# carrenD/Medical-Cross-Modality-Domain-Adaptation

Hardware: AMD Instinct MI355X
Metric: training slices/sec (256x256x3, B=16/GPU) joint segmenter+GAN step (1 dis update on B MR + B CT, clip, 1 gen update on B CT) (higher is better)
Workload: dtype f32; 1 GPU; BASELINE configs[3]: train_gan.py --phase train-gan joint step, B=16/GPU per domain, f32, dropout .75, mask critic on; global_batch=16, per_gpu_batch=16, parallelism=dp1, step_capture=False

## Files before the change

### include/pnp_hip.h

```cpp
#ifndef PNP_HIP_H
#define PNP_HIP_H

#include <stddef.h>
#include <stdint.h>

#ifdef __cplusplus
extern "C" {
#endif

#define PNP_OK 0
#define PNP_EINVAL (-1)
#define PNP_ELAUNCH (-2)
#define PNP_EWORKSPACE (-3)
#define PNP_ECOMM (-4)

#define PNP_DTYPE_F32 0
#define PNP_DTYPE_BF16 1
#define PNP_DTYPE_F64 2

#define PNP_PAD_ZERO 0
#define PNP_PAD_SYMMETRIC 1

int pnp_abi_version(void);
const char* pnp_last_error(void);
int pnp_device_info(int device, int* cu_count, int* clock_khz, int* lds_bytes, char* arch, int arch_len);

#define PNP_PROF_CONV_FWD 1
#define PNP_PROF_CONV_DGRAD 2
#define PNP_PROF_CONV_WGRAD 4
#define PNP_PROF_CONV_DIRECT 8
typedef struct pnp_prof_row {
    char name[128];
    int64_t launches;
    double ms, flops, bytes;
} pnp_prof_row;
int pnp_prof_enable(int32_t mask);
int pnp_prof_summary(pnp_prof_row* rows, int32_t max_rows);

typedef struct pnp_conv_geom {
    int32_t N, H, W, C;
    int32_t K, R, S;
    int32_t OH, OW;
    int32_t stride, dil;
    int32_t pad_t, pad_l;
    int32_t pad_mode;
    int32_t dtype;
} pnp_conv_geom;

int pnp_conv2d_fwd(const float* x, const float* w, float* y, const pnp_conv_geom* g,
                   float keep_prob, uint64_t seed, uint32_t stream_id, void* stream);
size_t pnp_conv2d_fwd_workspace_bytes(const pnp_conv_geom* g);
int pnp_conv2d_fwd_ws(const float* x, const float* w, float* y, const pnp_conv_geom* g,
                      float keep_prob, uint64_t seed, uint32_t stream_id,
                      void* workspace, size_t workspace_bytes, void* stream);

int32_t pnp_conv2d_fwd_stats_parts(const pnp_conv_geom* g);
int pnp_conv2d_fwd_stats(const float* x, const float* w, float* y, const pnp_conv_geom* g,
                         float keep_prob, uint64_t seed, uint32_t stream_id,
                         const float* shift , float* parts, size_t parts_bytes, void* stream);
int32_t pnp_conv2d_fwd_stats_ws_parts(const pnp_conv_geom* g);
int pnp_conv2d_fwd_stats_ws(const float* x, const float* w, float* y, const pnp_conv_geom* g,
                            float keep_prob, uint64_t seed, uint32_t stream_id,
                            const float* shift , float* parts, size_t parts_bytes,
                            void* workspace, size_t workspace_bytes, void* stream);
int32_t pnp_conv2d_wino_chosen(const pnp_conv_geom* g, int32_t kind);
#define PNP_ROUTE_IGEMM 0
#define PNP_ROUTE_N16 1
#define PNP_ROUTE_NARROW 2
#define PNP_ROUTE_WINO 3
#define PNP_ROUTE_X3D 4
#define PNP_ROUTE_X3S 5
#define PNP_ROUTE_PHASES 6
#define PNP_ROUTE_WINO_WGRAD 7
#define PNP_ROUTE_X3W 8
#define PNP_ROUTE_N16_WGRAD 9
#define PNP_ROUTE_WGD 10
#define PNP_ROUTE_RING 11
#define PNP_ROUTE_X3N 12
int32_t pnp_conv2d_route(const pnp_conv_geom* g, int32_t kind);
int32_t pnp_conv2d_wino_mode(int32_t mode);
int32_t pnp_conv2d_wino_tile(int32_t tile);
int32_t pnp_conv2d_wino_x3(int32_t mode);
int32_t pnp_conv2d_x3_direct(int32_t mode);
int32_t pnp_conv2d_x3_strided(int32_t mode);
int32_t pnp_conv2d_x3_wgrad(int32_t mode);
int32_t pnp_conv2d_x3_narrow(int32_t mode);
size_t pnp_conv2d_wino_filter_bytes(int32_t C, int32_t K);
int pnp_conv2d_wino_filter_bind(const float* w, int32_t kind, float* U, size_t bytes);
void pnp_weights_changed(const void* lo, const void* hi);
void pnp_conv2d_wino_filter_stats(int64_t* hits, int64_t* fills, int32_t reset);
int32_t pnp_conv2d_wino_wgrad_mode(int32_t mode);

int pnp_bn_fold(const float* gamma, const float* beta, const float* mean, const float* var, float* scale, float* shift,
                int32_t C, float eps, void* stream);
int pnp_conv2d_fwd_bn(const float* x, const float* w, float* y, const pnp_conv_geom* g,
                      float keep_prob, uint64_t seed, uint32_t stream_id,
                      const float* scale, const float* shift, const float* shortcut , int32_t Cs, float alpha,
                      void* stream);
int pnp_conv2d_fwd_bn_ws(const float* x, const float* w, float* y, const pnp_conv_geom* g,
                         float keep_prob, uint64_t seed, uint32_t stream_id,
                         const float* scale, const float* shift, const float* shortcut , int32_t Cs, float alpha,
                         void* workspace, size_t workspace_bytes, void* stream);

size_t pnp_conv2d_dgrad_workspace_bytes(const pnp_conv_geom* g);
int pnp_conv2d_dgrad(const float* dy, const float* w, float* dx, const pnp_conv_geom* g,
                     void* workspace, size_t workspace_bytes, void* stream);
int pnp_conv2d_dgrad_add(const float* dy, const float* w, const float* residual, float* dx, const pnp_conv_geom* g,
                         void* workspace, size_t workspace_bytes, void* stream);

size_t pnp_conv2d_wgrad_workspace_bytes(const pnp_conv_geom* g);
int pnp_conv2d_wgrad(const float* x, const float* dy, float* dw, const pnp_conv_geom* g,
                     void* workspace, size_t workspace_bytes, void* stream);
int pnp_conv2d_wgrad_acc(const float* x, const float* dy, float* dw, const pnp_conv_geom* g,
                         void* workspace, size_t workspace_bytes, void* stream);

int pnp_conv2d_fwd_naive(const float* x, const float* w, float* y, const pnp_conv_geom* g, void* stream);

int pnp_dropout(const float* x, float* y, size_t n, float keep_prob, uint64_t seed, uint32_t stream_id, void* stream);

size_t pnp_bn_workspace_bytes(int64_t P, int32_t C);
int pnp_bn_stats(const float* x, float* mean, float* var, int64_t P, int32_t C,
                 void* workspace, size_t workspace_bytes, void* stream);
int pnp_bn_stats_update(const float* x, float* mean, float* var, float* moving_mean, float* moving_var, int64_t P, int32_t C,
                        float decay, void* workspace, size_t workspace_bytes, void* stream);
int pnp_bn_stats_finish(float* parts, int32_t nparts, const float* shift, float* mean, float* var,
                        float* moving_mean, float* moving_var, int64_t P, int32_t C, float decay, void* stream);
int pnp_bn_update_moving(float* moving_mean, float* moving_var, const float* mean, const float* var,
                         int64_t P, int32_t C, float decay, void* stream);
int pnp_bn_apply(const float* x, const float* mean, const float* var, const float* gamma, const float* beta,
                 const float* shortcut, int32_t Cs, float* y, int64_t P, int32_t C, float eps, float alpha,
                 void* stream);
int pnp_bn_bwd(const float* dout, const float* out , const float* x, const float* mean, const float* var,
               const float* gamma, const float* beta , float* dx, float* dgamma, float* dbeta, float* dshortcut, int32_t Cs,
               int64_t P, int32_t C, float eps, float alpha, int32_t training,
               float keep_prob, uint64_t seed, uint32_t stream_id,
               void* workspace, size_t workspace_bytes, void* stream);
int pnp_bn_bwd_acc(const float* dout, const float* out , const float* x, const float* mean, const float* var,
                   const float* gamma, const float* beta , float* dx, float* dgamma, float* dbeta, float* dgamma_acc, float* dbeta_acc,
                   float* dshortcut, int32_t Cs, int64_t P, int32_t C, float eps, float alpha, int32_t training,
                   float keep_prob, uint64_t seed, uint32_t stream_id,
                   void* workspace, size_t workspace_bytes, void* stream);
int pnp_bn_bwd_reduce(const float* dout, const float* out , const float* x, const float* mean, const float* var,
                      const float* gamma , const float* beta , float* dgamma, float* dbeta, int64_t P, int32_t C, float eps, float alpha,
                      void* workspace, size_t workspace_bytes, void* stream);
int pnp_bn_bwd_apply(const float* dout, const float* out , const float* x, const float* mean, const float* var,
                     const float* gamma, const float* beta , const float* dgamma, const float* dbeta, float* dx, float* dshortcut, int32_t Cs,
                     int64_t P, int64_t P_norm, int32_t C, float eps, float alpha, int32_t training,
                     float keep_prob, uint64_t seed, uint32_t stream_id, void* stream);


int pnp_maxpool2_fwd(const float* x, float* y, int32_t N, int32_t H, int32_t W, int32_t C, void* stream);
int pnp_maxpool2_bwd(const float* x, const float* dy, float* dx, int32_t N, int32_t H, int32_t W, int32_t C, void* stream);

int pnp_ps_fwd(const float* x, float* y, int32_t N, int32_t A, int32_t B, int32_t r, int32_t nc, void* stream);
int pnp_ps_bwd(const float* dy, float* dx, int32_t N, int32_t A, int32_t B, int32_t r, int32_t nc, void* stream);

int pnp_sympad_fwd(const float* x, float* xp, int32_t N, int32_t H, int32_t W, int32_t C, int32_t p, void* stream);
int pnp_sympad_bwd(const float* dxp, float* dx, int32_t N, int32_t H, int32_t W, int32_t C, int32_t p, void* stream);

int pnp_ps_pad_fwd(const float* x, float* xp, int32_t N, int32_t A, int32_t B, int32_t r, int32_t nc, int32_t p, void* stream);
int pnp_ps_pad_bwd(const float* dxp, float* dx, int32_t N, int32_t A, int32_t B, int32_t r, int32_t nc, int32_t p, void* stream);

size_t pnp_seg_loss_workspace_bytes(int64_t P, int32_t ncls);
int pnp_seg_loss_fwd(const float* logits, const float* y, float* out, int64_t P, int32_t ncls,
                     float miu_cross, float miu_dice, void* workspace, size_t workspace_bytes, void* stream);
int pnp_seg_loss_bwd(const float* logits, const float* y, float* dlogits, int64_t P, int32_t ncls,
                     float miu_cross, float miu_dice, float gscale,
                     const void* workspace, size_t workspace_bytes, void* stream);
int pnp_seg_loss_bwd_norm(const float* logits, const float* y, float* dlogits, int64_t P, int64_t P_norm, int32_t ncls,
                          float miu_cross, float miu_dice, float gscale,
                          const void* workspace, size_t workspace_bytes, void* stream);
int pnp_softmax_argmax(const float* logits, float* prob , int64_t* label, int64_t P, int32_t ncls, void* stream);
int pnp_dice_eval(const int64_t* label, const float* y, float* out, int64_t P, int32_t ncls,
                  void* workspace, size_t workspace_bytes, void* stream);

int pnp_label_decomp(const float* label, float* onehot, int64_t P, int32_t ncls, void* stream);
int pnp_confusion_matrix(const float* y, const int64_t* pred, int64_t* compact_y, int64_t* cm, int64_t P, int32_t ncls, void* stream);
int pnp_edt3d_sq(const uint8_t* mask, float* dist_sq, int64_t X, int64_t Y, int64_t Z, float sx, float sy, float sz, void* stream);
size_t pnp_surface_workspace_bytes(int64_t X, int64_t Y, int64_t Z, int32_t ncls);
int pnp_surface_distances(const int32_t* pred, const int32_t* gt, int64_t X, int64_t Y, int64_t Z, int32_t ncls, float sx, float sy,
                          float sz, double* out, void* workspace, size_t workspace_bytes, void* stream);
int pnp_gp_interpolate(const float* a, const float* b, float* out, float* eps, int64_t B, int64_t n, uint64_t seed, uint32_t stream_id,
                       void* stream);
size_t pnp_gp_workspace_bytes(int64_t B, int64_t n);
int pnp_gp_penalty(float* g, int64_t B, int64_t n, float coef, float gscale, float* norms, float* penalty, void* workspace,
// ... 187 lines not shown
```

### medical-cross-modality-domain-adaptation_amd/_lib.py

```python
import ctypes
import os

import torch

from ctypes import POINTER, c_char_p, c_double, c_float, c_int, c_int32, c_int64, c_size_t, c_uint32, c_uint64, c_void_p

_HERE = os.path.dirname(os.path.abspath(__file__))
LIB_PATH = os.environ.get("PNP_LIB") or os.path.join(_HERE, "libpnp_hip.so")

PAD_ZERO = 0
PAD_SYMMETRIC = 1
OPT_CHUNK = 1024
DTYPE_F32, DTYPE_BF16, DTYPE_F64 = 0, 1, 2
COMM_ID_BYTES = 128
(ROUTE_IGEMM, ROUTE_N16, ROUTE_NARROW, ROUTE_WINO, ROUTE_X3D, ROUTE_X3S, ROUTE_PHASES,
 ROUTE_WINO_WGRAD, ROUTE_X3W, ROUTE_N16_WGRAD, ROUTE_WGD, ROUTE_RING, ROUTE_X3N) = range(13)
ABI_VERSION = 4


class ConvGeom(ctypes.Structure):
    _fields_ = [(n, c_int32) for n in
                ("N", "H", "W", "C", "K", "R", "S", "OH", "OW", "stride", "dil", "pad_t", "pad_l", "pad_mode", "dtype")]

    def key(self):
        return tuple(getattr(self, f) for f, _ in self._fields_)


class ProfRow(ctypes.Structure):
    _fields_ = [("name", ctypes.c_char * 128), ("launches", c_int64), ("ms", ctypes.c_double), ("flops", ctypes.c_double),
                ("bytes", ctypes.c_double)]


class AugVolume(ctypes.Structure):
    _fields_ = [("image", c_void_p), ("label", c_void_p), ("X", c_int32), ("Y", c_int32), ("Z", c_int32), ("fill", c_float)]


class AugSample(ctypes.Structure):
    _fields_ = [("volume", c_int32), ("frame", c_int32), ("m", c_float * 6)]


class AugSampleZ(ctypes.Structure):
    _fields_ = [("volume", c_int32), ("frame", c_int32), ("dz", c_float), ("m", c_float * 6)]


class AugSampleW(ctypes.Structure):
    _fields_ = [("volume", c_int32), ("frame", c_int32), ("dz", c_float), ("m", c_float * 6), ("gain", c_float), ("bias", c_float),
                ("noise", c_float), ("seed", c_uint32), ("warp", c_int32)]


PROF_CONV_FWD, PROF_CONV_DGRAD, PROF_CONV_WGRAD, PROF_CONV_DIRECT = 1, 2, 4, 8


class PnpError(RuntimeError):
    pass


_F = c_void_p
_G = POINTER(ConvGeom)

PROTOTYPES = {
    "pnp_abi_version": (c_int, []),
    "pnp_last_error": (c_char_p, []),
    "pnp_device_info": (c_int, [c_int, POINTER(c_int), POINTER(c_int), POINTER(c_int), c_char_p, c_int]),
    "pnp_prof_enable": (c_int, [c_int32]),
    "pnp_prof_summary": (c_int, [POINTER(ProfRow), c_int32]),
    "pnp_conv2d_fwd": (c_int, [_F, _F, _F, _G, c_float, c_uint64, c_uint32, c_void_p]),
    "pnp_conv2d_dgrad_workspace_bytes": (c_size_t, [_G]),
    "pnp_conv2d_dgrad": (c_int, [_F, _F, _F, _G, c_void_p, c_size_t, c_void_p]),
    "pnp_conv2d_dgrad_add": (c_int, [_F, _F, _F, _F, _G, c_void_p, c_size_t, c_void_p]),
    "pnp_conv2d_wgrad_workspace_bytes": (c_size_t, [_G]),
    "pnp_conv2d_wgrad": (c_int, [_F, _F, _F, _G, c_void_p, c_size_t, c_void_p]),
    "pnp_conv2d_wgrad_acc": (c_int, [_F, _F, _F, _G, c_void_p, c_size_t, c_void_p]),
    "pnp_conv2d_fwd_workspace_bytes": (c_size_t, [_G]),
    "pnp_conv2d_fwd_ws": (c_int, [_F, _F, _F, _G, c_float, c_uint64, c_uint32, c_void_p, c_size_t, c_void_p]),
    "pnp_conv2d_fwd_stats_parts": (c_int32, [_G]),
    "pnp_conv2d_fwd_stats": (c_int, [_F, _F, _F, _G, c_float, c_uint64, c_uint32, _F, _F, c_size_t, c_void_p]),
    "pnp_bn_stats_finish": (c_int, [_F, c_int32, _F, _F, _F, _F, _F, c_int64, c_int32, c_float, c_void_p]),
    "pnp_bn_fold": (c_int, [_F, _F, _F, _F, _F, _F, c_int32, c_float, c_void_p]),
    "pnp_conv2d_fwd_bn": (c_int, [_F, _F, _F, _G, c_float, c_uint64, c_uint32, _F, _F, _F, c_int32, c_float, c_void_p]),
    "pnp_conv2d_fwd_bn_ws": (c_int, [_F, _F, _F, _G, c_float, c_uint64, c_uint32, _F, _F, _F, c_int32, c_float, c_void_p, c_size_t, c_void_p]),
    "pnp_conv2d_fwd_stats_ws_parts": (c_int32, [_G]),
    "pnp_conv2d_fwd_stats_ws": (c_int, [_F, _F, _F, _G, c_float, c_uint64, c_uint32, _F, _F, c_size_t, c_void_p, c_size_t, c_void_p]),
    "pnp_conv2d_wino_chosen": (c_int32, [_G, c_int32]),
    "pnp_conv2d_route": (c_int32, [_G, c_int32]),
    "pnp_conv2d_wino_mode": (c_int32, [c_int32]),
    "pnp_conv2d_wino_wgrad_mode": (c_int32, [c_int32]),
    "pnp_conv2d_wino_tile": (c_int32, [c_int32]),
    "pnp_conv2d_wino_x3": (c_int32, [c_int32]),
    "pnp_conv2d_x3_direct": (c_int32, [c_int32]),
    "pnp_conv2d_x3_strided": (c_int32, [c_int32]),
    "pnp_conv2d_x3_wgrad": (c_int32, [c_int32]),
    "pnp_conv2d_x3_narrow": (c_int32, [c_int32]),
    "pnp_conv2d_wino_filter_bytes": (c_size_t, [c_int32, c_int32]),
    "pnp_conv2d_wino_filter_bind": (c_int, [c_void_p, c_int32, c_void_p, c_size_t]),
    "pnp_weights_changed": (None, [c_void_p, c_void_p]),
    "pnp_conv2d_wino_filter_stats": (None, [POINTER(c_int64), POINTER(c_int64), c_int32]),
    "pnp_conv2d_fwd_naive": (c_int, [_F, _F, _F, _G, c_void_p]),
    "pnp_dropout": (c_int, [_F, _F, c_size_t, c_float, c_uint64, c_uint32, c_void_p]),
    "pnp_bn_workspace_bytes": (c_size_t, [c_int64, c_int32]),
    "pnp_bn_stats": (c_int, [_F, _F, _F, c_int64, c_int32, c_void_p, c_size_t, c_void_p]),
    "pnp_bn_stats_update": (c_int, [_F, _F, _F, _F, _F, c_int64, c_int32, c_float, c_void_p, c_size_t, c_void_p]),
    "pnp_bn_update_moving": (c_int, [_F, _F, _F, _F, c_int64, c_int32, c_float, c_void_p]),
    "pnp_bn_apply": (c_int, [_F, _F, _F, _F, _F, _F, c_int32, _F, c_int64, c_int32, c_float, c_float, c_void_p]),
    "pnp_bn_bwd": (c_int, [_F, _F, _F, _F, _F, _F, _F, _F, _F, _F, _F, c_int32, c_int64, c_int32, c_float, c_float, c_int32,
                           c_float, c_uint64, c_uint32, c_void_p, c_size_t, c_void_p]),
    "pnp_bn_bwd_acc": (c_int, [_F, _F, _F, _F, _F, _F, _F, _F, _F, _F, _F, _F, _F, c_int32, c_int64, c_int32, c_float, c_float, c_int32,
                               c_float, c_uint64, c_uint32, c_void_p, c_size_t, c_void_p]),
    "pnp_bn_bwd_reduce": (c_int, [_F, _F, _F, _F, _F, _F, _F, _F, _F, c_int64, c_int32, c_float, c_float, c_void_p, c_size_t, c_void_p]),
    "pnp_bn_bwd_apply": (c_int, [_F, _F, _F, _F, _F, _F, _F, _F, _F, _F, _F, c_int32, c_int64, c_int64, c_int32, c_float, c_float, c_int32,
                                 c_float, c_uint64, c_uint32, c_void_p]),
    "pnp_maxpool2_fwd": (c_int, [_F, _F, c_int32, c_int32, c_int32, c_int32, c_void_p]),
    "pnp_maxpool2_bwd": (c_int, [_F, _F, _F, c_int32, c_int32, c_int32, c_int32, c_void_p]),
    "pnp_ps_fwd": (c_int, [_F, _F, c_int32, c_int32, c_int32, c_int32, c_int32, c_void_p]),
    "pnp_ps_bwd": (c_int, [_F, _F, c_int32, c_int32, c_int32, c_int32, c_int32, c_void_p]),
    "pnp_sympad_fwd": (c_int, [_F, _F, c_int32, c_int32, c_int32, c_int32, c_int32, c_void_p]),
    "pnp_sympad_bwd": (c_int, [_F, _F, c_int32, c_int32, c_int32, c_int32, c_int32, c_void_p]),
    "pnp_ps_pad_fwd": (c_int, [_F, _F, c_int32, c_int32, c_int32, c_int32, c_int32, c_int32, c_void_p]),
    "pnp_ps_pad_bwd": (c_int, [_F, _F, c_int32, c_int32, c_int32, c_int32, c_int32, c_int32, c_void_p]),
    "pnp_seg_loss_workspace_bytes": (c_size_t, [c_int64, c_int32]),
    "pnp_seg_loss_fwd": (c_int, [_F, _F, _F, c_int64, c_int32, c_float, c_float, c_void_p, c_size_t, c_void_p]),
    "pnp_seg_loss_bwd": (c_int, [_F, _F, _F, c_int64, c_int32, c_float, c_float, c_float, c_void_p, c_size_t, c_void_p]),
    "pnp_seg_loss_bwd_norm": (c_int, [_F, _F, _F, c_int64, c_int64, c_int32, c_float, c_float, c_float, c_void_p, c_size_t, c_void_p]),
    "pnp_softmax_argmax": (c_int, [_F, _F, c_void_p, c_int64, c_int32, c_void_p]),
    "pnp_dice_eval": (c_int, [c_void_p, _F, _F, c_int64, c_int32, c_void_p, c_size_t, c_void_p]),
    "pnp_adam_step": (c_int, [_F, _F, _F, _F, c_size_t, _F, c_void_p, c_float, c_float, c_float, c_float, c_int32, c_void_p]),
    "pnp_rmsprop_step": (c_int, [_F, _F, _F, c_size_t, _F, c_void_p, c_float, c_float, c_float, c_void_p]),
    "pnp_momentum_step": (c_int, [_F, _F, _F, c_size_t, _F, c_void_p, c_float, c_float, c_void_p]),
    "pnp_clip": (c_int, [_F, c_size_t, c_void_p, c_float, c_float, c_void_p]),
    "pnp_l2_loss": (c_int, [_F, c_size_t, _F, _F, c_void_p, c_size_t, c_void_p]),
    "pnp_reduce_workspace_bytes": (c_size_t, [c_size_t]),
    "pnp_critic_input_fwd": (c_int, [_F, c_int32, c_int32, _F, c_int32, _F, c_int32, _F, c_int32, _F, c_int32, _F, c_int64, c_void_p]),
    "pnp_critic_input_bwd": (c_int, [_F, _F, c_int32, c_int32, _F, c_int32, _F, c_int32, _F, c_int32, _F, c_int32, c_int64, c_void_p]),
    "pnp_critic_input_ps_fwd": (c_int, [_F, c_int32, c_int32, _F, c_int32, _F, c_int32, _F, c_int32, _F, c_int32, _F, c_int32, c_int32, c_int32,
                                        c_int32, c_void_p]),
    "pnp_critic_input_ps_bwd": (c_int, [_F, _F, c_int32, c_int32, _F, c_int32, _F, c_int32, _F, c_int32, _F, c_int32, c_int32, c_int32, c_int32,
                                        c_int32, c_void_p]),
    "pnp_axpby": (c_int, [_F, _F, c_size_t, c_float, c_float, c_void_p]),
    "pnp_add": (c_int, [_F, _F, _F, c_size_t, c_void_p]),
    "pnp_softmax_entropy_workspace_bytes": (c_size_t, [c_int64, c_int32]),
    "pnp_softmax_entropy": (c_int, [_F, c_int64, c_int32, c_float, _F, _F, c_void_p, c_size_t, c_void_p]),
    "pnp_signed_distance_2d_workspace_bytes": (c_size_t, [c_int32, c_int32, c_int32, c_int32, c_uint32]),
    "pnp_signed_distance_2d": (c_int, [_F, c_int32, c_int32, c_int32, c_int32, c_uint32, _F, c_void_p, c_size_t, c_void_p]),
    "pnp_boundary_loss_workspace_bytes": (c_size_t, [c_int64, c_int32]),
    "pnp_boundary_loss": (c_int, [_F, _F, c_int64, c_int32, c_int32, c_float, _F, _F, c_void_p, c_size_t, c_void_p]),
    "pnp_pseudo_label_loss_workspace_bytes": (c_size_t, [c_int64, c_int32]),
    "pnp_pseudo_label_loss": (c_int, [_F, _F, c_int64, c_int32, c_uint32, c_float, _F, c_void_p, _F, _F, c_void_p, c_void_p, c_size_t, c_void_p]),
    "pnp_pseudo_label_update_workspace_bytes": (c_size_t, [c_int64, c_int32]),
    "pnp_pseudo_label_update": (c_int, [c_void_p, _F, c_int64, c_int32, c_double, c_float, _F, _F, c_void_p, c_size_t, c_void_p]),
    "pnp_fda_workspace_bytes": (c_size_t, [c_int32, c_int32, c_int32, c_int32, c_int32, c_int32]),
    "pnp_fda_amplitude_swap": (c_int, [_F, c_int32, _F, c_int32, c_int32, c_int32, c_int32, c_void_p, c_void_p, _F, c_void_p, c_size_t, c_void_p]),
    "pnp_wgan_loss": (c_int, [_F, _F, _F, _F, c_int32, c_float, c_float, c_float, c_float, _F, c_void_p]),
    "pnp_fill": (c_int, [_F, c_size_t, c_float, c_void_p]),
    "pnp_label_decomp": (c_int, [_F, _F, c_int64, c_int32, c_void_p]),
    "pnp_confusion_matrix": (c_int, [_F, c_void_p, c_void_p, c_void_p, c_int64, c_int32, c_void_p]),
    "pnp_edt3d_sq": (c_int, [c_void_p, _F, c_int64, c_int64, c_int64, c_float, c_float, c_float, c_void_p]),
    "pnp_surface_workspace_bytes": (c_size_t, [c_int64, c_int64, c_int64, c_int32]),
    "pnp_surface_distances": (c_int, [c_void_p, c_void_p, c_int64, c_int64, c_int64, c_int32, c_float, c_float, c_float, c_void_p, c_void_p,
                                      c_size_t, c_void_p]),
    "pnp_gp_interpolate": (c_int, [_F, _F, _F, _F, c_int64, c_int64, c_uint64, c_uint32, c_void_p]),
    "pnp_gp_workspace_bytes": (c_size_t, [c_int64, c_int64]),
    "pnp_gp_penalty": (c_int, [_F, c_int64, c_int64, c_float, c_float, _F, _F, c_void_p, c_size_t, c_void_p]),
    "pnp_bn_dbl_bwd_workspace_bytes": (c_size_t, [c_int64, c_int32]),
    "pnp_bn_dbl_bwd": (c_int, [_F, _F, _F, _F, _F, _F, _F, _F, c_int32, _F, _F, _F, c_int64, c_int32, c_float, c_float, c_float, c_uint64,
                               c_uint32, c_void_p, c_size_t, c_void_p]),
    "pnp_bn_moments": (c_int, [_F, _F, c_void_p, c_int32, c_void_p]),
    "pnp_bn_from_moments": (c_int, [c_void_p, c_int32, _F, _F, c_int32, c_void_p]),
    "pnp_cast_bf16": (c_int, [_F, c_void_p, c_size_t, c_void_p]),
    "pnp_filter_bf16": (c_int, [_F, c_void_p, c_void_p, c_int32, c_int32, c_int32, c_int32, c_void_p]),
    "pnp_conv2d_bf16r_served": (c_int32, [_G, c_int32]),
    "pnp_conv2d_fwd_bf16r_stats_parts": (c_int32, [_G]),
    "pnp_conv2d_fwd_bf16r": (c_int, [c_void_p, c_void_p, _F, c_void_p, _G, c_float, c_uint64, c_uint32, _F, _F, c_size_t, _F, _F, _F, c_int32,
                                     c_float, c_void_p]),
    "pnp_conv2d_dgrad_bf16r": (c_int, [c_void_p, c_void_p, _F, _F, c_void_p, _G, c_void_p]),
    "pnp_bn_apply_h": (c_int, [_F, _F, _F, _F, _F, _F, c_int32, _F, c_void_p, c_int64, c_int32, c_float, c_float, c_void_p]),
    "pnp_bn_bwd_acc_h": (c_int, [_F, _F, _F, _F, _F, _F, _F, _F, c_void_p, _F, _F, _F, _F, _F, c_int32, c_int64, c_int32, c_float, c_float,
                                 c_int32, c_float, c_uint64, c_uint32, c_void_p, c_size_t, c_void_p]),
    "pnp_bn_bwd_apply_h": (c_int, [_F, _F, _F, _F, _F, _F, _F, _F, _F, _F, c_void_p, _F, c_int32, c_int64, c_int64, c_int32, c_float, c_float,
                                   c_int32, c_float, c_uint64, c_uint32, c_void_p]),
    "pnp_dropout_h": (c_int, [_F, _F, c_void_p, c_size_t, c_float, c_uint64, c_uint32, c_void_p]),
# ... 87 lines not shown
```

### medical-cross-modality-domain-adaptation_amd/csrc/conv_common.h

```cpp
#pragma once
#include "pnp_common.h"

namespace pnpconv {

constexpr int BK = 32;
constexpr int NTHREADS = 256;

struct ConvArgs {
    const float* x;
    const float* w;
    float* y;
    int N, H, W, C, K, R, S, OH, OW, stride, dil, pad_t, pad_l, pad_mode;
    int ups;
    int M;
    int Kred;
    int OHW;
    int nblk_m, nblk_n;
    int gn;
    int nsplit, chunks_per_split;
    long long split_stride;
    uint32_t drop_thresh, drop_key;
    float drop_keep;
    int do_drop;
    const pnp_step_params* sp;
    uint32_t drop_sid;
    int xcd_swizzle;
    unsigned x_bytes, w_bytes;
    int stagger;
    int o_s, o_H, o_W, o_h0, o_w0;
    const float* ep_scale;
    const float* ep_shift;
    const float* ep_res;
    int ep_cs;
    float ep_alpha;
    int dtype;
    float* stat_ws;
    const float* stat_shift;
    const float* res_add;
    int accumulate;
    int ow_sh, ohw_sh;
    int ph_st, ph_pa, ph_pb, ph_S;
    unsigned short* y_h;
};

__device__ __forceinline__ void split_row(const ConvArgs& a, int m, int& n, int& oh, int& ow) {
    if (a.ohw_sh >= 0) {
        n = m >> a.ohw_sh;
        const int rem = m & (a.OHW - 1);
        oh = rem >> a.ow_sh;
        ow = rem & (a.OW - 1);
    } else {
        n = m / a.OHW;
        const int rem = m - n * a.OHW;
        oh = rem / a.OW;
        ow = rem - oh * a.OW;
    }
}

__device__ __forceinline__ float bn_epilogue(const ConvArgs& a, float v, int m, int n) {
    v = fmaf(v, a.ep_scale[n], a.ep_shift[n]);
    if (a.ep_res) {
        const int cs = n - ((a.K - a.ep_cs) >> 1);
        if ((unsigned)cs < (unsigned)a.ep_cs) v += a.ep_res[(size_t)m * a.ep_cs + cs];
    }
    return (a.ep_alpha >= 0.f && v < 0.f) ? v * a.ep_alpha : v;
}

__device__ __forceinline__ size_t out_row(const ConvArgs& a, int m, bool scatter) {
    if (!scatter) return (size_t)m * a.K;
    int n, oh, ow;
    split_row(a, m, n, oh, ow);
    return ((size_t)(n * a.o_H + a.o_h0 + oh * a.o_s) * a.o_W + a.o_w0 + ow * a.o_s) * a.K;
}

template <bool UPS>
__device__ __forceinline__ bool map_coord(int v, int H, int ups, int sym, int& i) {
    const int vs = v < 0 ? -1 - v : (v >= H ? 2 * H - 1 - v : v);
    const int vv = sym ? vs : v;
    if constexpr (UPS) {
        const int q = vv / ups;
        i = q;
        return (vv >= 0) & (q * ups == vv) & (q < H);
    } else {
        i = vv;
        return (unsigned)vv < (unsigned)H;
    }
}

__device__ __forceinline__ int xcd_remap(int bid, int nblk) {
    const int NX = 8;
    int q = nblk / NX, r = nblk % NX;
    int xcd = bid % NX, idx = bid / NX;
    int base = (xcd < r) ? xcd * (q + 1) : r * (q + 1) + (xcd - r) * q;
    return base + idx;
}

__device__ __forceinline__ void tile_coords(int bid, int nblk_m, int nblk_n, int gn, int& mt, int& nt) {
    if (gn <= 0 || gn >= nblk_n) { mt = bid / nblk_n; nt = bid - mt * nblk_n; return; }
    const int span = nblk_m * gn;
    const int sc = bid / span, rem = bid - sc * span;
    const int left = nblk_n - sc * gn;
    const int width = left < gn ? left : gn;
    mt = rem / width;
    nt = sc * gn + rem - mt * width;
}

template <int TM, int TN>
struct Acc {
    f32x16 v[TM][TN];
    __device__ __forceinline__ void zero() {
#pragma unroll
        for (int i = 0; i < TM; ++i)
#pragma unroll
            for (int j = 0; j < TN; ++j)
#pragma unroll
                for (int e = 0; e < 16; ++e) v[i][j][e] = 0.f;
    }
};

typedef unsigned int u32x4 __attribute__((ext_vector_type(4)));
typedef const float __attribute__((address_space(4))) pnp_cfloat;
constexpr unsigned OOB = 0xFFFFFF00u;

__device__ __forceinline__ __amdgpu_buffer_rsrc_t make_rsrc(const float* p, unsigned bytes) {
    return __builtin_amdgcn_make_buffer_rsrc(const_cast<float*>(p), 0, bytes, 0x00020000);
}
__device__ __forceinline__ f32x4 bload4(__amdgpu_buffer_rsrc_t r, unsigned off) {
    return __builtin_bit_cast(f32x4, __builtin_amdgcn_raw_buffer_load_b128(r, off, 0, 0));
}
__device__ __forceinline__ float bload1(__amdgpu_buffer_rsrc_t r, unsigned off) {
    return __builtin_bit_cast(float, __builtin_amdgcn_raw_buffer_load_b32(r, off, 0, 0));
}
__device__ __forceinline__ void bstore1(__amdgpu_buffer_rsrc_t r, unsigned off, float v) {
    __builtin_amdgcn_raw_buffer_store_b32(__builtin_bit_cast(unsigned, v), r, off, 0, 0);
}


template <int TM, int TN>
__device__ __forceinline__ void conv_epilogue(const ConvArgs& a, const Acc<TM, TN>& acc, float* __restrict__ yout, int m0, int n0, int wm0,
                                              int wn0, int lane, int part, bool first_split = true) {
    const float* __restrict__ res = first_split ? a.res_add : nullptr;
    const int l31 = lane & 31, h = lane >> 5;
    const bool scatter = a.o_s != 0 && a.nsplit == 1;
// ... 117 lines not shown
        for (int tm = 0; tm < TM; ++tm)
#pragma unroll
            for (int tn = 0; tn < TN; ++tn) {
                const int n = n0 + wn0 + tn * 32 + l31;
#pragma unroll
                for (int r = 0; r < 16; ++r) {
                    const int m = mbase + tm * 32 + (r & 3) + 8 * (r >> 2);
                    const bool ok = (m < a.Kred) & (n < a.K);
                    old.v[tm][tn][r] = out[ok ? (size_t)m * a.K + n : 0];
                }
            }
#pragma unroll
        for (int tm = 0; tm < TM; ++tm)
#pragma unroll
            for (int tn = 0; tn < TN; ++tn)
#pragma unroll
                for (int r = 0; r < 16; ++r) o.v[tm][tn][r] += old.v[tm][tn][r];
    }
#pragma unroll
    for (int tm = 0; tm < TM; ++tm)
#pragma unroll
        for (int tn = 0; tn < TN; ++tn) {
            const int n = n0 + wn0 + tn * 32 + l31;
#pragma unroll
            for (int r = 0; r < 16; ++r) {
                const int m = mbase + tm * 32 + (r & 3) + 8 * (r >> 2);
                if ((m < a.Kred) & (n < a.K)) out[(size_t)m * a.K + n] = o.v[tm][tn][r];
            }
        }
}

constexpr unsigned OOB2 = 0x80000000u;

__device__ __forceinline__ f32x4 bload4s(__amdgpu_buffer_rsrc_t r, unsigned voff, int soff) {
    return __builtin_bit_cast(f32x4, __builtin_amdgcn_raw_buffer_load_b128(r, voff, soff, 0));
}

__device__ __forceinline__ float bload1s(__amdgpu_buffer_rsrc_t r, unsigned voff, int soff) {
    return __builtin_bit_cast(float, __builtin_amdgcn_raw_buffer_load_b32(r, voff, soff, 0));
}

bool launch_taps_bf16(const ConvArgs& a, int tile, int kind, dim3 grid, hipStream_t st);
bool launch_wgrad_bf16(const ConvArgs& a, int tile, dim3 grid, hipStream_t st);
constexpr int kWgradBf16rChunk = 64;
bool launch_wgrad_bf16r(const ConvArgs& a, int tile, dim3 grid, hipStream_t st);
int wgrad_bf16r_tile(const pnp_conv_geom* g);
struct DgradPhase {
    int pa, pb, T, U, h0, w0, I, J, pad_t, pad_l;
    size_t wt_off;
};
int plan_phases(const pnp_conv_geom* g, DgradPhase* ph);
pnp_conv_geom phase_geom(const pnp_conv_geom* g, const DgradPhase& p);
bool n16_geom_ok(const pnp_conv_geom* g);
bool n16_wgrad_ok(const pnp_conv_geom* g);
int launch_n16_fwd(const ConvArgs& a, int kind, hipStream_t st);
int n16_wgrad_blocks(const pnp_conv_geom* g);
int launch_n16_wgrad(const ConvArgs& a, float* part, hipStream_t st);
bool narrow_fwd_ok(const pnp_conv_geom* g);
int launch_narrow(const float* x, const float* w, float* y, const pnp_conv_geom* g, const ConvArgs& a, hipStream_t st);
bool wgd_ok(const pnp_conv_geom* g);
size_t wgd_workspace_bytes(const pnp_conv_geom* g);
int wgd_blocks(const pnp_conv_geom* g);
int launch_wgd(const float* x, const float* dy, float* part, const pnp_conv_geom* g, const ConvArgs& a, hipStream_t st);
bool x3d_chosen(const pnp_conv_geom* g);
int x3d_stats_parts(const pnp_conv_geom* g);
size_t x3d_filter_bytes(int C, int K);
int launch_x3_direct(const ConvArgs& a, int kind, bool flip_transpose, void* ws, size_t ws_bytes, hipStream_t st);
bool x3s_chosen(const pnp_conv_geom* g, int kind);
size_t x3s_filter_bytes(const pnp_conv_geom* g);
int launch_x3_strided(const ConvArgs& a, const pnp_conv_geom* g, int kind, void* ws, size_t ws_bytes, hipStream_t st);
int x3d_route_mode();
bool x3w_chosen(const pnp_conv_geom* g);
size_t x3w_workspace_bytes(const pnp_conv_geom* g);
int launch_x3_wgrad(const float* x, const float* dy, float* dw, const pnp_conv_geom* g, int accumulate, void* ws, size_t ws_bytes, hipStream_t st);
bool x3n_chosen(const pnp_conv_geom* g, int kind);
size_t x3n_filter_bytes(int kind);
int launch_x3_narrow(const ConvArgs& a, int kind, void* ws, size_t ws_bytes, hipStream_t st);
struct WinoQuery {
    int tile;
    size_t ws_bytes;
    int stats_parts;
};
WinoQuery wino_query(const pnp_conv_geom* g);
int launch_wino(const ConvArgs& a, int kind, bool flip_transpose, void* ws, size_t ws_bytes, hipStream_t st);
WinoQuery wino_wgrad_query(const pnp_conv_geom* g);
int launch_wino_wgrad(const ConvArgs& a, float* dw, int accumulate, void* ws, size_t ws_bytes, hipStream_t st);
#ifndef PNP_X3_SW
#define PNP_X3_SW 32
#endif
constexpr int X3_SW = PNP_X3_SW;
static_assert(X3_SW == 16 || X3_SW == 32, "stage width");
bool wino_x3_dims_ok(int T, int C, int K);
int launch_wino_gemm_x3(const unsigned short* V3, const unsigned short* U3, float* Mm, int T, int C, int K, int npos, int sym, int gn, int xcd,
                        int nsplit, int stages_per_split, hipStream_t st);
inline double conv_flops(const ConvArgs& a) { return 2.0 * (double)a.M * a.K * a.Kred; }
inline double conv_bytes(const ConvArgs& a) {
    return 4.0 * ((double)a.N * a.H * a.W * a.C + (double)a.M * a.K + (double)a.Kred * a.K);
}
inline int prof_class(int kind) { return kind == 0 ? PNP_PROF_CONV_FWD : PNP_PROF_CONV_DGRAD; }

}
```

### medical-cross-modality-domain-adaptation_amd/csrc/conv_igemm.hip

```cpp
#include "conv_common.h"
#include "conv_mma.h"
#include "split_sum.h"

using namespace pnpconv;

#ifdef PNP_TRACE
constexpr int TRACE_WG = 512, TRACE_N = 192;
__device__ unsigned long long g_trace[TRACE_WG][TRACE_N];
#define PNP_TRACE_MARK(slot)                                                                             \
    do {                                                                                                 \
        const unsigned tr_ = blockIdx.x - (gridDim.x > 4352u ? 4096u : 0u);        \
        if (threadIdx.x == 0 && tr_ < (unsigned)TRACE_WG && (slot) < TRACE_N) g_trace[tr_][(slot)] = __builtin_readcyclecounter(); \
    } while (0)
extern "C" int pnp_debug_trace_read(void* host, size_t bytes) {
    if (bytes > sizeof(unsigned long long) * TRACE_WG * TRACE_N) bytes = sizeof(unsigned long long) * TRACE_WG * TRACE_N;
    return hipMemcpyFromSymbol(host, HIP_SYMBOL(g_trace), bytes, 0, hipMemcpyDeviceToHost) == hipSuccess ? 0 : -1;
}
#else
#define PNP_TRACE_MARK(slot) do { } while (0)
#endif

namespace {

template <int BN, bool VEC>
// ... 766 lines not shown
    Stage ring[DEPTH];
    int l_chunk = c_begin;
    auto gload = [&](Stage& st) {
#pragma unroll
        for (int i = 0; i < ANP; ++i) {
            if constexpr (UNI) {
                unsigned so[2];
#pragma unroll
                for (int h = 0; h < 2; ++h) {
                    const bool ok = ((unsigned)u_ih[i][h] < (unsigned)a.H) & ((unsigned)u_iw[i][h] < (unsigned)a.W);
                    so[h] = ok ? (unsigned)u_off[i][h] : OOB2;
                    u_iw[i][h] += step_w;
                    u_ih[i][h] += step_h;
                    u_off[i][h] += step_off;
                    const bool ww = u_iw[i][h] >= u_iw_lim;
                    u_iw[i][h] -= ww ? wrap_w : 0;
                    u_ih[i][h] += ww ? a.stride : 0;
                    u_off[i][h] += ww ? wrap_w_off : 0;
                    const bool hw = u_ih[i][h] >= u_ih_lim;
                    u_ih[i][h] -= hw ? wrap_h : 0;
                    u_off[i][h] += hw ? wrap_h_off : 0;
                }
                st.a[i] = bload4(rx, ((lane & 32) ? so[1] : so[0]) + lane_c);
                continue;
            }
            const bool ok = mok & ((unsigned)l_ih[i] < (unsigned)a.H) & ((unsigned)l_iw[i] < (unsigned)a.W);
            st.a[i] = bload4(rx, ok ? (unsigned)l_off[i] : OOB);
            l_iw[i] += step_w;
            l_ih[i] += step_h;
            l_off[i] += step_off;
            const bool ww = l_iw[i] >= iw_lim;
            l_iw[i] -= ww ? wrap_w : 0;
            l_ih[i] += ww ? a.stride : 0;
            l_off[i] += ww ? wrap_w_off : 0;
            const bool hw = l_ih[i] >= ih_lim;
            l_ih[i] -= hw ? wrap_h : 0;
            l_off[i] += hw ? wrap_h_off : 0;
        }
        const int soff = __builtin_amdgcn_readfirstlane(l_chunk * BK * a.K * 4);
#pragma unroll
        for (int i = 0; i < BNP; ++i) st.b[i] = bload4s(rw, boff[i], soff);
        l_chunk = (l_chunk + 1 < nchunks_total) ? l_chunk + 1 : nchunks_total;
    };
    auto lstore = [&](const Stage& st, float* An, float* Bn) {
#pragma unroll
        for (int i = 0; i < ANP; ++i) *reinterpret_cast<f32x4*>(An + (arow + ARP * i) * LDA + 4 * acol) = st.a[i];
#pragma unroll
        for (int i = 0; i < BNP; ++i) *reinterpret_cast<f32x4*>(Bn + (brow + BRP * i) * LDB + 4 * bcol) = st.b[i];
    };

    Acc<TM, TN> acc;
    acc.zero();
    if (nchunks > 0) {
#pragma unroll
        for (int d = 0; d < DEPTH; ++d) gload(ring[d]);
        lstore(ring[0], lds, lds + 2 * ASZ);
        __syncthreads();
        Frag<TM, TN, false, LDA, LDB> f0, f1;
        f0.load(lds, lds + 2 * ASZ, 0, wm0, wn0, lane);
        auto stage = [&](int j, Stage& fetch_into, const Stage& store_from, bool fetch) {
            const int cur = j & 1;
            const float* As = lds + cur * ASZ;
            const float* Bs = lds + 2 * ASZ + cur * BSZ;
            float* An = lds + (cur ^ 1) * ASZ;
            float* Bn = lds + 2 * ASZ + (cur ^ 1) * BSZ;
            PNP_MMA_STAGE(12, 4 * TM + 4 * TN, 4 * TM * TN, if (fetch) gload(fetch_into), lstore(store_from, An, Bn))
            f0.load(An, Bn, 0, wm0, wn0, lane);
        };
        const int nmain = (nchunks / DEPTH) * DEPTH;
        for (int j0 = 0; j0 < nmain; j0 += DEPTH) {
#pragma unroll
            for (int d = 0; d < DEPTH; ++d) stage(j0 + d, ring[d], ring[(d + 1) % DEPTH], true);
        }
        if (nchunks - nmain >= 1) stage(nmain, ring[0], ring[1], false);
    }

    wgrad_epilogue<TM, TN>(a, acc, a.y + (size_t)z * a.split_stride, mm0, n0, wm0, wn0, lane);
}

__global__ void bn_fold_kernel(const float* __restrict__ gamma, const float* __restrict__ beta, const float* __restrict__ mean,
                               const float* __restrict__ var, float* __restrict__ scale, float* __restrict__ shift, int C, float eps) {
    const int c = blockIdx.x * blockDim.x + threadIdx.x;
    if (c >= C) return;
    const float sc = gamma[c] * (1.0f / sqrtf(var[c] + eps));
    scale[c] = sc;
    shift[c] = beta[c] - mean[c] * sc;
}

__global__ void flip_transpose_phase_kernel(const float* __restrict__ w, float* __restrict__ wt, int R, int S, int C, int K, int st) {
    __shared__ float tile[32][33];
    const int r = blockIdx.z / S, sx = blockIdx.z - r * S;
    const int pa = r % st, pb = sx % st;
    const int T = (R - pa + st - 1) / st, U = (S - pb + st - 1) / st;
    int taps_before = 0;
    for (int a = 0; a < st; ++a)
        for (int b = 0; b < st; ++b)
            if (a * st + b < pa * st + pb) taps_before += ((R - a + st - 1) / st) * ((S - b + st - 1) / st);
    const int tf = T - 1 - r / st, uf = U - 1 - sx / st;
    const float* src = w + (size_t)blockIdx.z * C * K;
    float* dst = wt + ((size_t)taps_before + tf * U + uf) * K * C;
    const int c0 = blockIdx.y * 32, k0 = blockIdx.x * 32;
    const int tx = threadIdx.x & 31, ty = threadIdx.x >> 5;
    for (int i = ty; i < 32; i += 8) {
        int c = c0 + i, k = k0 + tx;
        tile[i][tx] = (c < C && k < K) ? src[(size_t)c * K + k] : 0.f;
    }
    __syncthreads();
    for (int i = ty; i < 32; i += 8) {
        int k = k0 + i, c = c0 + tx;
        if (k < K && c < C) dst[(size_t)k * C + c] = tile[tx][i];
    }
}

__global__ void flip_transpose_kernel(const float* __restrict__ w, float* __restrict__ wt, int R, int S, int C, int K) {
    __shared__ float tile[32][33];
    const int rs = blockIdx.z;
    const int r = rs / S, s = rs - r * S;
    const int rs_f = (R - 1 - r) * S + (S - 1 - s);
    const float* src = w + (size_t)rs * C * K;
    float* dst = wt + (size_t)rs_f * K * C;
    const int c0 = blockIdx.y * 32, k0 = blockIdx.x * 32;
    const int tx = threadIdx.x & 31, ty = threadIdx.x >> 5;
    for (int i = ty; i < 32; i += 8) {
        int c = c0 + i, k = k0 + tx;
        tile[i][tx] = (c < C && k < K) ? src[(size_t)c * K + k] : 0.f;
    }
    __syncthreads();
    for (int i = ty; i < 32; i += 8) {
        int k = k0 + i, c = c0 + tx;
        if (k < K && c < C) dst[(size_t)k * C + c] = tile[tx][i];
    }
}

__global__ void naive_conv_kernel(ConvArgs a) {
    size_t idx = (size_t)blockIdx.x * blockDim.x + threadIdx.x;
    const size_t total = (size_t)a.M * a.K;
    if (idx >= total) return;
    const int k = (int)(idx % a.K);
    const int m = (int)(idx / a.K);
    const int n = m / a.OHW;
    const int rem = m - n * a.OHW;
    const int oh = rem / a.OW, ow = rem - oh * a.OW;
    float acc = 0.f;
    for (int r = 0; r < a.R; ++r)
        for (int s = 0; s < a.S; ++s) {
            int ih = 0, iw = 0;
            if (!map_coord<true>(oh * a.stride - a.pad_t + r * a.dil, a.H, a.ups, a.pad_mode, ih)) continue;
            if (!map_coord<true>(ow * a.stride - a.pad_l + s * a.dil, a.W, a.ups, a.pad_mode, iw)) continue;
            const float* xp = a.x + ((size_t)(n * a.H + ih) * a.W + iw) * a.C;
            const float* wp = a.w + (size_t)((r * a.S + s) * a.C) * a.K + k;
            for (int c = 0; c < a.C; ++c) acc = fmaf(xp[c], wp[(size_t)c * a.K], acc);
        }
    a.y[idx] = acc;
}

__global__ void sympad_fwd_kernel(const float* __restrict__ x, float* __restrict__ xp, int N, int H, int W, int C, int p, int vec) {
    const int CV = vec ? (C >> 2) : C;
    const int Hp = H + 2 * p, Wp = W + 2 * p;
    const size_t total = (size_t)N * Hp * Wp * CV;
    const size_t gs = (size_t)gridDim.x * blockDim.x;
    for (size_t i = (size_t)blockIdx.x * blockDim.x + threadIdx.x; i < total; i += gs) {
        const int cv = (int)(i % CV);
        size_t q = i / CV;
        const int wp = (int)(q % Wp);
        q /= Wp;
        const int hp = (int)(q % Hp);
        const int n = (int)(q / Hp);
        int h = hp - p, w = wp - p;
        h = h < 0 ? -1 - h : (h >= H ? 2 * H - 1 - h : h);
// ... 522 lines not shown
    int route;
    size_t x3 = 0;
    DgradPhase ph[16];
    const int nph = plan_phases(g, ph);
    p.dws = dgrad_ws(g, d, ph, nph);
    const size_t b = p.dws.total;
    if (nph > 0) {
        route = x3s_chosen(g, 1) ? PNP_ROUTE_X3S : PNP_ROUTE_PHASES;
        if (route == PNP_ROUTE_X3S) x3 = x3s_filter_bytes(g);
    } else {
        if (!sym && n16_geom_ok(&d)) route = PNP_ROUTE_N16;
        else if (g->stride == 1 && narrow_fwd_ok(&d)) route = PNP_ROUTE_NARROW;
        else if (plain && x3d_chosen(&d)) route = PNP_ROUTE_X3D;
        else if (plain && x3n_chosen(g, 1)) route = PNP_ROUTE_X3N;
        else route = PNP_ROUTE_IGEMM;
        if (route == PNP_ROUTE_X3D) x3 = x3d_filter_bytes(d.C, d.K);
        if (route == PNP_ROUTE_X3N) x3 = x3n_filter_bytes(1);
    }
    p.ws_bytes = b > x3 ? b : x3;
    p.add(route, p.ws_bytes);
    return p;
}

static ConvPlan plan_wgrad(const pnp_conv_geom* g) {
    ConvPlan p{};
    const WinoQuery wq = wino_wgrad_query(g);
    p.tile = wq.tile;
    if (p.tile) p.add(PNP_ROUTE_WINO_WGRAD, wq.ws_bytes);
    if (x3w_chosen(g)) p.add(PNP_ROUTE_X3W, x3w_workspace_bytes(g));
    const size_t nout = (size_t)g->R * g->S * g->C * g->K;
    const bool wgd = wgd_ok(g);
    const int nsplit = ring_split(g);
    if (p.ncand) p.ws_bytes = p.cand[0].need;
    else if (n16_wgrad_ok(g)) p.ws_bytes = (size_t)n16_wgrad_blocks(g) * nout * sizeof(float);
    else {
        const size_t mfma_ws = nsplit <= 1 ? 0 : (size_t)nsplit * nout * sizeof(float);
        p.ws_bytes = (wgd && wgd_workspace_bytes(g) > mfma_ws) ? wgd_workspace_bytes(g) : mfma_ws;
    }
    if (n16_wgrad_ok(g)) p.add(PNP_ROUTE_N16_WGRAD, p.ws_bytes);
    if (wgd) p.add(PNP_ROUTE_WGD, wgd_workspace_bytes(g));
    p.add(PNP_ROUTE_RING, 0, nsplit);
    return p;
}

static void set_dropout(ConvArgs& a, float keep_prob, uint64_t seed, uint32_t stream_id) {
    if (keep_prob >= 1.f) return;
    a.do_drop = 1;
    a.drop_keep = keep_prob;
    a.drop_key = pnp_drop_key(seed, stream_id);
    a.drop_thresh = pnp_drop_thresh(keep_prob);
    a.sp = pnp_step_params_ptr(); a.drop_sid = stream_id;
}

static int launch_fwd_cand(const ConvPlan::Cand& c, ConvArgs& a, const pnp_conv_geom* g, void* ws, size_t ws_bytes, hipStream_t st) {
    switch (c.route) {
    case PNP_ROUTE_N16: return launch_n16_fwd(a, 0, st);
    case PNP_ROUTE_NARROW: return launch_narrow(a.x, a.w, a.y, g, a, st);
    case PNP_ROUTE_WINO: return launch_wino(a, 0, false, ws, ws_bytes, st);
    case PNP_ROUTE_X3D: return launch_x3_direct(a, 0, false, ws, ws_bytes, st);
    case PNP_ROUTE_X3S: return launch_x3_strided(a, g, 0, ws, ws_bytes, st);
    case PNP_ROUTE_X3N: return launch_x3_narrow(a, 0, ws, ws_bytes, st);
    default: return launch_fwd<0>(a, st, c.need ? (float*)ws : nullptr, ws_bytes, c.nsplit);
    }
}

static ConvPlan plan_of(const pnp_conv_geom* g, int kind) { return kind == 0 ? plan_fwd(g, EP_WS) : (kind == 2 ? plan_wgrad(g) : plan_dgrad(g)); }

extern "C" {

int32_t pnp_conv2d_route(const pnp_conv_geom* g, int32_t kind) {
    if (!g || check_geom(g, "pnp_conv2d_route") != PNP_OK) return -1;
    return plan_of(g, kind).cand[0].route;
}

int32_t pnp_conv2d_wino_chosen(const pnp_conv_geom* g, int32_t kind) {
    if (!g || check_geom(g, "pnp_conv2d_wino_chosen") != PNP_OK) return 0;
    return plan_of(g, kind).tile;
}

size_t pnp_conv2d_fwd_workspace_bytes(const pnp_conv_geom* g) { return g ? plan_fwd(g, EP_WS).ws_bytes : 0; }
size_t pnp_conv2d_dgrad_workspace_bytes(const pnp_conv_geom* g) { return g ? plan_dgrad(g).ws_bytes : 0; }
size_t pnp_conv2d_wgrad_workspace_bytes(const pnp_conv_geom* g) { return g ? plan_wgrad(g).ws_bytes : 0; }

int pnp_conv2d_fwd(const float* x, const float* w, float* y, const pnp_conv_geom* g, float keep_prob, uint64_t seed,
                   uint32_t stream_id, void* stream) {
    return pnp_conv2d_fwd_ws(x, w, y, g, keep_prob, seed, stream_id, nullptr, 0, stream);
}

int pnp_conv2d_fwd_ws(const float* x, const float* w, float* y, const pnp_conv_geom* g, float keep_prob, uint64_t seed,
                      uint32_t stream_id, void* workspace, size_t workspace_bytes, void* stream) {
    if (int e = check_geom(g, "pnp_conv2d_fwd")) return e;
    PNP_REQUIRE(x && w && y, "pnp_conv2d_fwd: null pointer");
    PNP_REQUIRE(keep_prob > 0.f, "pnp_conv2d_fwd: keep_prob must be > 0");
    ConvArgs a = make_args(x, w, y, g);
    set_dropout(a, keep_prob, seed, stream_id);
    return launch_fwd_cand(plan_fwd(g, EP_WS).pick(workspace, workspace_bytes), a, g, workspace, workspace_bytes, (hipStream_t)stream);
}

static int fwd_stats_impl(const float* x, const float* w, float* y, const pnp_conv_geom* g, float keep_prob, uint64_t seed,
                          uint32_t stream_id, const float* shift, float* parts, size_t parts_bytes, void* workspace, size_t workspace_bytes,
                          void* stream, unsigned ep) {
    if (int e = check_geom(g, "pnp_conv2d_fwd_stats")) return e;
    PNP_REQUIRE(x && w && y && parts, "pnp_conv2d_fwd_stats: null pointer");
    PNP_REQUIRE(keep_prob > 0.f, "pnp_conv2d_fwd_stats: keep_prob must be > 0");
    const ConvPlan p = plan_fwd(g, ep);
    const ConvPlan::Cand& c = p.cand[0];
    PNP_REQUIRE(c.need == 0 || (workspace && workspace_bytes >= c.need), "pnp_conv2d_fwd_stats_ws: workspace too small (pnp_conv2d_fwd_workspace_bytes)");
    PNP_REQUIRE(p.stats_parts > 0, "pnp_conv2d_fwd_stats: no epilogue statistics for this geometry (pnp_conv2d_fwd_stats_parts == 0)");
    if (parts_bytes < (size_t)p.stats_parts * 2 * g->K * sizeof(float)) {
        pnp_set_error("pnp_conv2d_fwd_stats: parts buffer too small (%zu < %zu)", parts_bytes, (size_t)p.stats_parts * 2 * g->K * sizeof(float));
        return PNP_EWORKSPACE;
    }
    ConvArgs a = make_args(x, w, y, g);
    set_dropout(a, keep_prob, seed, stream_id);
    a.stat_ws = parts;
    a.stat_shift = shift;
    return launch_fwd_cand(c, a, g, workspace, workspace_bytes, (hipStream_t)stream);
}

int32_t pnp_conv2d_fwd_stats_parts(const pnp_conv_geom* g) {
    return (g && check_geom(g, "pnp_conv2d_fwd_stats_parts") == PNP_OK) ? plan_fwd(g, EP_STATS).stats_parts : 0;
}

int pnp_conv2d_fwd_stats(const float* x, const float* w, float* y, const pnp_conv_geom* g, float keep_prob, uint64_t seed,
                         uint32_t stream_id, const float* shift, float* parts, size_t parts_bytes, void* stream) {
    return fwd_stats_impl(x, w, y, g, keep_prob, seed, stream_id, shift, parts, parts_bytes, nullptr, 0, stream, EP_STATS);
}

int32_t pnp_conv2d_fwd_stats_ws_parts(const pnp_conv_geom* g) {
    return (g && check_geom(g, "pnp_conv2d_fwd_stats_ws_parts") == PNP_OK) ? plan_fwd(g, EP_STATS | EP_WS).stats_parts : 0;
}

int pnp_conv2d_fwd_stats_ws(const float* x, const float* w, float* y, const pnp_conv_geom* g, float keep_prob, uint64_t seed,
                            uint32_t stream_id, const float* shift, float* parts, size_t parts_bytes, void* workspace,
                            size_t workspace_bytes, void* stream) {
    return fwd_stats_impl(x, w, y, g, keep_prob, seed, stream_id, shift, parts, parts_bytes, workspace, workspace_bytes, stream, EP_STATS | EP_WS);
}

int pnp_bn_fold(const float* gamma, const float* beta, const float* mean, const float* var, float* scale, float* shift, int32_t C,
                float eps, void* stream) {
    PNP_REQUIRE(gamma && beta && mean && var && scale && shift && C > 0, "pnp_bn_fold: bad argument");
    hipLaunchKernelGGL(bn_fold_kernel, dim3((unsigned)pnp_cdiv(C, 256)), dim3(256), 0, (hipStream_t)stream, gamma, beta, mean, var, scale,
                       shift, C, eps);
    PNP_CHECK_LAUNCH("bn_fold_kernel");
    return PNP_OK;
}

int pnp_conv2d_fwd_bn(const float* x, const float* w, float* y, const pnp_conv_geom* g, float keep_prob, uint64_t seed,
                      uint32_t stream_id, const float* scale, const float* shift, const float* shortcut, int32_t Cs, float alpha,
                      void* stream) {
    return pnp_conv2d_fwd_bn_ws(x, w, y, g, keep_prob, seed, stream_id, scale, shift, shortcut, Cs, alpha, nullptr, 0, stream);
}

int pnp_conv2d_fwd_bn_ws(const float* x, const float* w, float* y, const pnp_conv_geom* g, float keep_prob, uint64_t seed,
                         uint32_t stream_id, const float* scale, const float* shift, const float* shortcut, int32_t Cs, float alpha,
                         void* workspace, size_t workspace_bytes, void* stream) {
    if (int e = check_geom(g, "pnp_conv2d_fwd_bn")) return e;
    PNP_REQUIRE(x && w && y && scale && shift, "pnp_conv2d_fwd_bn: null pointer");
    PNP_REQUIRE(keep_prob > 0.f, "pnp_conv2d_fwd_bn: keep_prob must be > 0");
    if (shortcut) PNP_REQUIRE(Cs > 0 && Cs <= g->K && ((g->K - Cs) % 2) == 0, "pnp_conv2d_fwd_bn: bad shortcut channels");
    ConvArgs a = make_args(x, w, y, g);
    set_dropout(a, keep_prob, seed, stream_id);
    a.ep_scale = scale; a.ep_shift = shift; a.ep_res = shortcut; a.ep_cs = shortcut ? Cs : g->K; a.ep_alpha = alpha;
    return launch_fwd_cand(plan_fwd(g, EP_WS | EP_BN).pick(workspace, workspace_bytes), a, g, workspace, workspace_bytes, (hipStream_t)stream);
}

int pnp_conv2d_fwd_naive(const float* x, const float* w, float* y, const pnp_conv_geom* g, void* stream) {
    if (int e = check_geom(g, "pnp_conv2d_fwd_naive")) return e;
    ConvArgs a = make_args(x, w, y, g);
    const size_t total = (size_t)a.M * a.K;
    hipLaunchKernelGGL(naive_conv_kernel, dim3((unsigned)pnp_cdiv((long long)total, 256)), dim3(256), 0,
                       (hipStream_t)stream, a);
    PNP_CHECK_LAUNCH("naive_conv_kernel");
    return PNP_OK;
}

static int dgrad_impl(const float* dy, const float* w, float* dx, const pnp_conv_geom* g, void* workspace, size_t workspace_bytes, void* stream,
                      const float* residual) {
    if (int e = check_geom(g, "pnp_conv2d_dgrad")) return e;
    PNP_REQUIRE(dy && w && dx && workspace, "pnp_conv2d_dgrad: null pointer");
    const ConvPlan p = plan_dgrad(g);
    PNP_REQUIRE(workspace_bytes >= p.ws_bytes, "pnp_conv2d_dgrad: workspace too small");
    const bool sym = g->pad_mode == PNP_PAD_SYMMETRIC;
    if (sym) PNP_REQUIRE(g->pad_t == g->pad_l, "pnp_conv2d_dgrad: SYMMETRIC needs pad_t == pad_l");
    hipStream_t st = (hipStream_t)stream;
    const int route = p.cand[0].route;
    const pnp_conv_geom d = dgrad_as_conv(g);
    if (route == PNP_ROUTE_X3S) {
        ConvArgs a = make_args(dy, w, dx, g);
        if (int e = launch_x3_strided(a, g, 1, workspace, workspace_bytes, st)) return e;
        return residual ? pnp_axpby(residual, dx, (size_t)g->N * g->H * g->W * g->C, 1.f, 1.f, stream) : PNP_OK;
    }
    if (route == PNP_ROUTE_WINO || route == PNP_ROUTE_X3D || route == PNP_ROUTE_X3N) {
        ConvArgs a = make_args(dy, w, dx, &d);
        a.res_add = residual;
        if (route == PNP_ROUTE_X3N) return launch_x3_narrow(a, 1, workspace, workspace_bytes, st);
        return route == PNP_ROUTE_WINO ? launch_wino(a, 1, true, workspace, workspace_bytes, st)
                                       : launch_x3_direct(a, 1, true, workspace, workspace_bytes, st);
    }
    const DgradWs& dws = p.dws;
    float* wt = (float*)workspace;
    float* out = sym ? (float*)((char*)workspace + dws.filt) : dx;
    float* parts = (float*)((char*)workspace + dws.filt + dws.padded);
    auto split_ws = [&](int ns) { return ns > 1 ? parts : nullptr; };
    const dim3 tg((unsigned)pnp_cdiv(g->K, 32), (unsigned)pnp_cdiv(g->C, 32), (unsigned)(g->R * g->S));
    if (route == PNP_ROUTE_PHASES) {
        DgradPhase ph[16];
        const int nph = plan_phases(g, ph);
        hipLaunchKernelGGL(flip_transpose_phase_kernel, tg, dim3(256), 0, st, w, wt, g->R, g->S, g->C, g->K, g->stride);
        PNP_CHECK_LAUNCH("flip_transpose_phase_kernel");
        if (phases_in_one_launch(g, ph, nph)) {
            if (int e = launch_phase_group(dy, wt, out, g, ph, nph, d.OH, d.OW, st)) return e;
        } else {
            for (int i = 0; i < nph; ++i) {
                const DgradPhase& q = ph[i];
                if (q.I == 0 || q.J == 0) continue;
                const pnp_conv_geom dp = phase_geom(g, q);
                ConvArgs a = make_args(dy, wt + q.wt_off, out, &dp);
                a.o_s = g->stride; a.o_H = d.OH; a.o_W = d.OW; a.o_h0 = q.h0; a.o_w0 = q.w0;
                if (int e = launch_fwd<1>(a, st, split_ws(dws.nsplit[i]), dws.parts, dws.nsplit[i])) return e;
            }
        }
    } else {
        hipLaunchKernelGGL(flip_transpose_kernel, tg, dim3(256), 0, st, w, wt, g->R, g->S, g->C, g->K);
        PNP_CHECK_LAUNCH("flip_transpose_kernel");
        PNP_REQUIRE(d.pad_t >= 0 && d.pad_l >= 0, "pnp_conv2d_dgrad: forward padding exceeds the filter extent");
        ConvArgs a = make_args(dy, wt, out, &d);
        a.ups = g->stride;
        if (route == PNP_ROUTE_N16) {
            a.res_add = residual;
            return launch_n16_fwd(a, 1, st);
        }
        if (route == PNP_ROUTE_NARROW) {
            if (int e = launch_narrow(dy, wt, out, &d, a, st)) return e;
        } else {
            if (residual && !sym && g->stride == 1) {
                a.res_add = residual;
                residual = nullptr;
            }
            const int ns = dws.nsplit[0];
            if (int e = (g->stride > 1 ? launch_fwd<2>(a, st, split_ws(ns), dws.parts, ns) : launch_fwd<1>(a, st, split_ws(ns), dws.parts, ns))) return e;
        }
    }
    if (sym) {
        if (int e = pnp_sympad_bwd(out, dx, g->N, g->H, g->W, g->C, g->pad_t, stream)) return e;
    }
    return residual ? pnp_axpby(residual, dx, (size_t)g->N * g->H * g->W * g->C, 1.f, 1.f, stream) : PNP_OK;
}

int pnp_conv2d_dgrad(const float* dy, const float* w, float* dx, const pnp_conv_geom* g, void* workspace,
                     size_t workspace_bytes, void* stream) {
    return dgrad_impl(dy, w, dx, g, workspace, workspace_bytes, stream, nullptr);
}

int pnp_conv2d_dgrad_add(const float* dy, const float* w, const float* residual, float* dx, const pnp_conv_geom* g, void* workspace,
                         size_t workspace_bytes, void* stream) {
    PNP_REQUIRE(residual && residual != dx, "pnp_conv2d_dgrad_add: residual must be a tensor of its own");
    return dgrad_impl(dy, w, dx, g, workspace, workspace_bytes, stream, residual);
}

static int wgrad_impl(const float* x, const float* dy, float* dw, const pnp_conv_geom* g, void* workspace, size_t workspace_bytes, void* stream,
                      int accumulate) {
    if (int e = check_geom(g, "pnp_conv2d_wgrad")) return e;
    PNP_REQUIRE(x && dy && dw, "pnp_conv2d_wgrad: null pointer");
    ConvArgs a = make_args(x, dy, dw, g);
    a.accumulate = accumulate;
    a.w_bytes = (unsigned)((size_t)g->N * g->OH * g->OW * g->K * sizeof(float));
    hipStream_t st = (hipStream_t)stream;
    float* ws = (float*)workspace;
    if (!ws) workspace_bytes = 0;
    const size_t nout = (size_t)a.Kred * a.K;
    int nparts = 0;
    const ConvPlan::Cand c = plan_wgrad(g).pick(workspace, workspace_bytes);
    switch (c.route) {
    case PNP_ROUTE_WINO_WGRAD: return launch_wino_wgrad(a, dw, accumulate, workspace, workspace_bytes, st);
    case PNP_ROUTE_X3W: return launch_x3_wgrad(x, dy, dw, g, accumulate, workspace, workspace_bytes, st);
    case PNP_ROUTE_N16_WGRAD:
        if (int e = launch_n16_wgrad(a, ws, st)) return e;
        nparts = n16_wgrad_blocks(g);
        break;
    case PNP_ROUTE_WGD:
        if (int e = launch_wgd(x, dy, ws, g, a, st)) return e;
        nparts = wgd_blocks(g);
        break;
    default: {
        const RingTile t = ring_tile(a.K);
        if (!t.vecb) return launch_wgrad_tile<128, 32, 4, 1, false>(a, dw, ws, workspace_bytes, c.nsplit, st);
        if (t.bn == 128) return launch_wgrad_tile<128, 128, 2, 2, true>(a, dw, ws, workspace_bytes, c.nsplit, st);
        if (t.bn == 64) return launch_wgrad_tile<128, 64, 2, 2, true>(a, dw, ws, workspace_bytes, c.nsplit, st);
        return launch_wgrad_tile<128, 32, 4, 1, true>(a, dw, ws, workspace_bytes, c.nsplit, st);
    }
    }
    return split_sum::launch_sliced<1>(ws, dw, (int)nout, nparts, accumulate, st);
}

int pnp_conv2d_wgrad(const float* x, const float* dy, float* dw, const pnp_conv_geom* g, void* workspace,
                     size_t workspace_bytes, void* stream) {
    return wgrad_impl(x, dy, dw, g, workspace, workspace_bytes, stream, 0);
}

int pnp_conv2d_wgrad_acc(const float* x, const float* dy, float* dw, const pnp_conv_geom* g, void* workspace,
                         size_t workspace_bytes, void* stream) {
    return wgrad_impl(x, dy, dw, g, workspace, workspace_bytes, stream, 1);
}

static int wgrad_bf16r_plan(const pnp_conv_geom* g, int* bm, int* bn) {
    const int tile = wgrad_bf16r_tile(g);
    if (tile < 0) return 0;
// ... 79 lines not shown
```

### medical-cross-modality-domain-adaptation_amd/csrc/conv_small.hip

```cpp
#include "conv_common.h"

using namespace pnpconv;

namespace {

constexpr int TH = 8, TW = 32;
constexpr int PH = TH + 2, PW = TW + 2;

__device__ __forceinline__ f32x4 mfma16(float a, float b, f32x4 c) { return __builtin_amdgcn_mfma_f32_16x16x4f32(a, b, c, 0, 0, 0); }

template <int C, int LD>
__device__ __forceinline__ void load_patch(const ConvArgs& a, __amdgpu_buffer_rsrc_t rx, float* __restrict__ lds, int n, int oh0, int ow0, int t) {
    constexpr int CQ = C / 4;
    for (int i = t; i < PH * PW * CQ; i += 256) {
        const int pix = i / CQ, cq = i - pix * CQ;
        const int py = pix / PW, px = pix - py * PW;
        const int ih = oh0 - a.pad_t + py, iw = ow0 - a.pad_l + px;
        const bool ok = ((unsigned)ih < (unsigned)a.H) & ((unsigned)iw < (unsigned)a.W);
        const f32x4 v = bload4(rx, ok ? (unsigned)((((n * a.H + ih) * a.W + iw) * C + 4 * cq) * 4) : OOB);
        *reinterpret_cast<f32x4*>(lds + pix * LD + 4 * cq) = v;
    }
}

template <int C, int KIND>
__global__ void __launch_bounds__(256) conv_n16_kernel(ConvArgs a, int tiles_w, int tiles_per_wg) {
    constexpr int LD = C + 4, NH = C / 16;
    __shared__ __attribute__((aligned(16))) float lds[PH * PW * LD];
    const int t = threadIdx.x, lane = t & 63;
    const int wave = __builtin_amdgcn_readfirstlane(t >> 6);
    const int p = lane & 15, g = lane >> 4;
    const int n = blockIdx.z, oh0 = blockIdx.y * TH;
    const __amdgpu_buffer_rsrc_t rx = make_rsrc(a.x, a.x_bytes);

    float wreg[9][NH][4];
#pragma unroll
    for (int tap = 0; tap < 9; ++tap)
#pragma unroll
        for (int h = 0; h < NH; ++h)
#pragma unroll
            for (int j = 0; j < 4; ++j) wreg[tap][h][j] = a.w[(tap * C + 16 * h + 4 * g + j) * 16 + p];

    const int jt0 = blockIdx.x * tiles_per_wg;
    for (int jt = jt0; jt < jt0 + tiles_per_wg && jt < tiles_w; ++jt) {
        const int ow0 = jt * TW;
        __syncthreads();
        load_patch<C, LD>(a, rx, lds, n, oh0, ow0, t);
        __syncthreads();
        f32x4 acc[4];
#pragma unroll
        for (int q = 0; q < 4; ++q) acc[q] = f32x4{0.f, 0.f, 0.f, 0.f};
#pragma unroll
        for (int tap = 0; tap < 9; ++tap) {
            const int r = tap / 3, s = tap % 3;
#pragma unroll
            for (int q = 0; q < 4; ++q) {
                const int pix = (2 * wave + (q >> 1) + r) * PW + 16 * (q & 1) + p + s;
#pragma unroll
                for (int h = 0; h < NH; ++h) {
                    const f32x4 av = *reinterpret_cast<const f32x4*>(lds + pix * LD + 16 * h + 4 * g);
#pragma unroll
                    for (int j = 0; j < 4; ++j) acc[q] = mfma16(av[j], wreg[tap][h][j], acc[q]);
                }
            }
        }
        float ov[4][4];
        size_t oidx[4][4];
        bool ook[4][4];
#pragma unroll
        for (int q = 0; q < 4; ++q) {
            const int oh = oh0 + 2 * wave + (q >> 1);
#pragma unroll
            for (int i = 0; i < 4; ++i) {
                const int ow = ow0 + 16 * (q & 1) + 4 * g + i;
                ook[q][i] = oh < a.OH && ow < a.OW;
                const int m = ook[q][i] ? (n * a.OH + oh) * a.OW + ow : 0;
                oidx[q][i] = (size_t)m * 16 + p;
                float v = acc[q][i];
                if (a.do_drop) v = pnp_drop_keep((uint32_t)oidx[q][i], pnp_eff_drop_key(a.drop_key, a.sp, a.drop_sid), a.drop_thresh) ? v / a.drop_keep : 0.f;
                if (a.res_add) v += a.res_add[oidx[q][i]];
                if (a.ep_scale) v = bn_epilogue(a, v, m, p);
                ov[q][i] = v;
            }
        }
#pragma unroll
        for (int q = 0; q < 4; ++q)
#pragma unroll
            for (int i = 0; i < 4; ++i)
                if (ook[q][i]) a.y[oidx[q][i]] = ov[q][i];
    }
}

template <int C>
__global__ void __launch_bounds__(256) wgrad_n16_kernel(ConvArgs a, int tiles_w, int tiles_h, int ntiles) {
    constexpr int LD = (C == 16) ? 16 : 48, NC = C / 16, NT = 9 * NC;
    constexpr int LDSF = PH * PW * LD > NT * 256 ? PH * PW * LD : NT * 256;
    __shared__ __attribute__((aligned(16))) float lds[LDSF];
    const int t = threadIdx.x, lane = t & 63;
    const int wave = __builtin_amdgcn_readfirstlane(t >> 6);
    const int p = lane & 15, g = lane >> 4;
    const __amdgpu_buffer_rsrc_t rx = make_rsrc(a.x, a.x_bytes);
    const __amdgpu_buffer_rsrc_t rdy = make_rsrc(a.w, a.w_bytes);
    const int kg0 = blockIdx.y * 16;
    f32x4 acc[NT];
#pragma unroll
    for (int i = 0; i < NT; ++i) acc[i] = f32x4{0.f, 0.f, 0.f, 0.f};

    for (int tile = blockIdx.x; tile < ntiles; tile += gridDim.x) {
        const int jt = tile % tiles_w, rest = tile / tiles_w;
        const int it = rest % tiles_h, n = rest / tiles_h;
        const int oh0 = it * TH, ow0 = jt * TW;
        __syncthreads();
        load_patch<C, LD>(a, rx, lds, n, oh0, ow0, t);
        __syncthreads();
#pragma unroll 4
        for (int q = 0; q < 16; ++q) {
            const int row = 2 * wave + (q >> 3), col = 4 * (q & 7) + g;
            const int oh = oh0 + row, ow = ow0 + col;
            const bool ok = (oh < a.OH) & (ow < a.OW);
            const float dyv = bload1(rdy, ok ? (unsigned)((((n * a.OH + oh) * a.OW + ow) * a.K + kg0 + p) * 4) : OOB);
#pragma unroll
            for (int tap = 0; tap < 9; ++tap) {
                const int pix = (row + tap / 3) * PW + col + tap % 3;
#pragma unroll
                for (int c = 0; c < NC; ++c) {
                    const float xv = lds[pix * LD + 16 * c + p];
                    acc[tap * NC + c] = mfma16(xv, dyv, acc[tap * NC + c]);
                }
            }
        }
    }
    for (int w = 0; w < 4; ++w) {
        __syncthreads();
        if (wave == w) {
#pragma unroll
            for (int i = 0; i < NT; ++i) {
                f32x4* slot = reinterpret_cast<f32x4*>(lds + (i * 64 + lane) * 4);
                if (w == 0) *slot = acc[i];
                else {
                    f32x4 v = *slot;
#pragma unroll
                    for (int k = 0; k < 4; ++k) v[k] += acc[i][k];
                    *slot = v;
                }
            }
        }
    }
    __syncthreads();
    float* out = a.y + (size_t)blockIdx.x * (9 * C * a.K) + kg0;
    for (int e = t; e < NT * 64; e += 256) {
        const int i = e >> 6, l = e & 63;
        const f32x4 s = *reinterpret_cast<const f32x4*>(lds + (i * 64 + l) * 4);
        const int tap = i / NC, c = i - tap * NC, lp = l & 15, lg = l >> 4;
#pragma unroll
        for (int k = 0; k < 4; ++k) out[(size_t)(tap * C + 16 * c + 4 * lg + k) * a.K + lp] = s[k];
    }
}

__device__ __forceinline__ void load_patch3(const ConvArgs& a, __amdgpu_buffer_rsrc_t rx, float* __restrict__ lds, int n, int oh0, int ow0, int t) {
    for (int i = t; i < PH * PW; i += 256) {
        const int py = i / PW, px = i - py * PW;
        const int ih = oh0 - a.pad_t + py, iw = ow0 - a.pad_l + px;
        const bool ok = ((unsigned)ih < (unsigned)a.H) & ((unsigned)iw < (unsigned)a.W);
        const unsigned off = ok ? (unsigned)((((n * a.H + ih) * a.W + iw) * 3) * 4) : OOB;
        f32x4 v;
        v[0] = bload1(rx, off);
        v[1] = bload1(rx, ok ? off + 4u : OOB);
        v[2] = bload1(rx, ok ? off + 8u : OOB);
        v[3] = 0.f;
        *reinterpret_cast<f32x4*>(lds + i * 4) = v;
    }
}

template <int KIND>
__global__ void __launch_bounds__(256) conv_c3n16_kernel(ConvArgs a, int tiles_w, int tiles_per_wg) {
    __shared__ __attribute__((aligned(16))) float lds[PH * PW * 4];
    const int t = threadIdx.x, lane = t & 63;
    const int wave = __builtin_amdgcn_readfirstlane(t >> 6);
    const int p = lane & 15, g = lane >> 4;
    const int n = blockIdx.z, oh0 = blockIdx.y * TH;
    const __amdgpu_buffer_rsrc_t rx = make_rsrc(a.x, a.x_bytes);
    float wreg[7];
    int aoff[7];
#pragma unroll
    for (int i = 0; i < 7; ++i) {
        const int kk = 4 * i + g;
        const int tap = kk < 27 ? kk / 3 : 0, c = kk < 27 ? kk - 3 * (kk / 3) : 3;
        wreg[i] = kk < 27 ? a.w[kk * 16 + p] : 0.f;
        aoff[i] = ((tap / 3) * PW + tap % 3) * 4 + c;
    }
    const int jt0 = blockIdx.x * tiles_per_wg;
    for (int jt = jt0; jt < jt0 + tiles_per_wg && jt < tiles_w; ++jt) {
        const int ow0 = jt * TW;
        __syncthreads();
        load_patch3(a, rx, lds, n, oh0, ow0, t);
        __syncthreads();
#pragma unroll
        for (int q = 0; q < 4; ++q) {
            const int base = ((2 * wave + (q >> 1)) * PW + 16 * (q & 1) + p) * 4;
            f32x4 acc = {0.f, 0.f, 0.f, 0.f};
#pragma unroll
            for (int i = 0; i < 7; ++i) acc = mfma16(lds[base + aoff[i]], wreg[i], acc);
            const int oh = oh0 + 2 * wave + (q >> 1);
            float ov[4];
            size_t oidx[4];
            bool ook[4];
#pragma unroll
            for (int i = 0; i < 4; ++i) {
                const int ow = ow0 + 16 * (q & 1) + 4 * g + i;
                ook[i] = oh < a.OH && ow < a.OW;
                const int m = ook[i] ? (n * a.OH + oh) * a.OW + ow : 0;
                oidx[i] = (size_t)m * 16 + p;
                float v = acc[i];
                if (a.do_drop) v = pnp_drop_keep((uint32_t)oidx[i], pnp_eff_drop_key(a.drop_key, a.sp, a.drop_sid), a.drop_thresh) ? v / a.drop_keep : 0.f;
                if (a.res_add) v += a.res_add[oidx[i]];
                if (a.ep_scale) v = bn_epilogue(a, v, m, p);
                ov[i] = v;
            }
#pragma unroll
            for (int i = 0; i < 4; ++i)
                if (ook[i]) a.y[oidx[i]] = ov[i];
        }
    }
}

__global__ void __launch_bounds__(256) wgrad_c3n16_kernel(ConvArgs a, int tiles_w, int tiles_h, int ntiles) {
    __shared__ __attribute__((aligned(16))) float lds[PH * PW * 4 > 2 * 256 ? PH * PW * 4 : 2 * 256];
    const int t = threadIdx.x, lane = t & 63;
    const int wave = __builtin_amdgcn_readfirstlane(t >> 6);
    const int p = lane & 15, g = lane >> 4;
    const __amdgpu_buffer_rsrc_t rx = make_rsrc(a.x, a.x_bytes);
    const __amdgpu_buffer_rsrc_t rdy = make_rsrc(a.w, a.w_bytes);
    int aoff[2];
#pragma unroll
    for (int T = 0; T < 2; ++T) {
        const int mm = 16 * T + p;
        const int tap = mm < 27 ? mm / 3 : 0, c = mm < 27 ? mm - 3 * (mm / 3) : 3;
        aoff[T] = ((tap / 3) * PW + tap % 3) * 4 + c;
    }
    f32x4 acc[2] = {{0.f, 0.f, 0.f, 0.f}, {0.f, 0.f, 0.f, 0.f}};
    for (int tile = blockIdx.x; tile < ntiles; tile += gridDim.x) {
        const int jt = tile % tiles_w, rest = tile / tiles_w;
        const int it = rest % tiles_h, n = rest / tiles_h;
        const int oh0 = it * TH, ow0 = jt * TW;
        __syncthreads();
        load_patch3(a, rx, lds, n, oh0, ow0, t);
        __syncthreads();
#pragma unroll 4
        for (int q = 0; q < 16; ++q) {
            const int row = 2 * wave + (q >> 3), col = 4 * (q & 7) + g;
            const int oh = oh0 + row, ow = ow0 + col;
            const bool ok = (oh < a.OH) & (ow < a.OW);
            const float dyv = bload1(rdy, ok ? (unsigned)((((n * a.OH + oh) * a.OW + ow) * 16 + p) * 4) : OOB);
            const int base = (row * PW + col) * 4;
            acc[0] = mfma16(lds[base + aoff[0]], dyv, acc[0]);
            acc[1] = mfma16(lds[base + aoff[1]], dyv, acc[1]);
        }
    }
    for (int w = 0; w < 4; ++w) {
        __syncthreads();
        if (wave == w) {
#pragma unroll
            for (int i = 0; i < 2; ++i) {
                f32x4* slot = reinterpret_cast<f32x4*>(lds + (i * 64 + lane) * 4);
                if (w == 0) *slot = acc[i];
                else {
                    f32x4 v = *slot;
#pragma unroll
                    for (int k = 0; k < 4; ++k) v[k] += acc[i][k];
                    *slot = v;
                }
            }
        }
    }
    __syncthreads();
    float* out = a.y + (size_t)blockIdx.x * (27 * 16);
    if (t < 128) {
        const int i = t >> 6, l = t & 63;
        const f32x4 s = *reinterpret_cast<const f32x4*>(lds + (i * 64 + l) * 4);
#pragma unroll
        for (int k = 0; k < 4; ++k) {
            const int mm = 16 * i + 4 * (l >> 4) + k;
            if (mm < 27) out[mm * 16 + (l & 15)] = s[k];
        }
    }
}

}

namespace pnpconv {

bool n16_geom_ok(const pnp_conv_geom* g) {
    static const int off = getenv("PNP_CONV_NON16") ? 1 : 0;
    if (off || g->K != 16 || (g->C != 16 && g->C != 32 && g->C != 3) || g->R != 3 || g->S != 3 || g->stride != 1 || g->dil != 1) return false;
    static const int f32only = getenv("PNP_N16_F32ONLY") ? 1 : 0;
    if (g->pad_mode != PNP_PAD_ZERO || g->pad_t > 1 || g->pad_l > 1 || (f32only && g->dtype != PNP_DTYPE_F32)) return false;
    if (g->OH != g->H + 2 * g->pad_t - 2 || g->OW != g->W + 2 * g->pad_l - 2) return false;
    return (long long)g->N * g->OH * g->OW >= 8192 && g->N <= 65535;
}
// ... 57 lines not shown
```

### medical-cross-modality-domain-adaptation_amd/csrc/conv_wino.hip

```cpp
#include <atomic>
#include <map>
#include <mutex>
#include "conv_x3_common.h"
#include "conv_mma.h"

using namespace pnpconv;

namespace {

constexpr int NT = 256;

__device__ __forceinline__ f32x4 ld4(const float* p) { return *reinterpret_cast<const f32x4*>(p); }
__device__ __forceinline__ void st4(float* p, f32x4 v) { *reinterpret_cast<f32x4*>(p) = v; }

__device__ __forceinline__ void st4x3(__bf16* p, size_t pstride, f32x4 v) {
    bf16x4 h, m, l;
    split3(v, h, m, l);
    store3(p, pstride * sizeof(__bf16), h, m, l);
}

struct WinoGeom {
    int N, Hi, Wi, Ho, Wo, dil, ps, Hsi, Wsi, Hso, Wso, th, tw, T;
    int m;
};
// ... 306 lines not shown
#pragma unroll
    for (int i = 0; i < NPB; ++i) breg[i] = bload4s(rw, boff[i], 0);
    lstore(lds, lds + 2 * ASZ);
    __syncthreads();
    Frag<TM, TN, true, LDA, LDB> f0, f1;
    f0.load(lds, lds + 2 * ASZ, 0, wm0, wn0, lane);
    int sidx = 0;
    int local = first;
    bool in_tail = false;
    for (;;) {
        const int nl = local + step;
        const bool next_whole = !in_tail && nl < whole_end;
        const bool next_tail = !in_tail && !next_whole && has_tail;
        const bool more = next_whole || next_tail;
        int cc0_n = 0;
        if (more) {
            setup(base + (next_whole ? nl : tail_tile), abase_n, boff_n, pos_n, m0_n, n0_n);
            cc0_n = next_tail ? tail_piece * cpp : 0;
        } else {
#pragma unroll
            for (int i = 0; i < NR; ++i) abase_n[i] = OOB2;
#pragma unroll
            for (int i = 0; i < NPB; ++i) boff_n[i] = OOB2;
        }
        const int cc_begin = in_tail ? tail_piece * cpp : 0, cc_end = in_tail ? cc_begin + cpp : ncc;
        for (int cc = cc_begin; cc < cc_end; ++cc, ++sidx) {
            const int cur = sidx & 1;
            const float* As = lds + cur * ASZ;
            const float* Bs = lds + 2 * ASZ + cur * BSZ;
            float* An = lds + (cur ^ 1) * ASZ;
            float* Bn = lds + 2 * ASZ + (cur ^ 1) * BSZ;
            const bool lastst = cc + 1 >= cc_end;
            const int cn = lastst ? cc0_n : cc + 1;
            const int sa = cn * (BK * 4);
            const int sb = (cn * BK * g.K) * 4;
            PNP_MMA_STAGE(4, 8, 4 * TM * TN,
                          _Pragma("unroll") for (int i = 0; i < NR; ++i) areg[i] = bload4s(rx, lastst ? abase_n[i] : abase[i], sa);
                          _Pragma("unroll") for (int i = 0; i < NPB; ++i) breg[i] = bload4s(rw, lastst ? boff_n[i] : boff[i], sb),
                          lstore(An, Bn))
            f0.load(An, Bn, 0, wm0, wn0, lane);
        }
        if (in_tail && tail_piece > 0) {
            const int x = g.xcd_swizzle ? (int)blockIdx.x % 8 : 0;
            ConvArgs ep{};
            ep.M = (g.T - m0 < BM) ? g.T - m0 : BM;
            ep.K = BN;
            ep.nsplit = 1;
            float* dst = g.Px + ((size_t)(x * g.tail_R + (tail_tile - g.tail_F)) * (split - 1) + (tail_piece - 1)) * (BM * BN);
            conv_epilogue<TM, TN>(ep, acc, dst, 0, 0, wm0, wn0, lane, 0);
        } else {
            conv_epilogue<TM, TN>(e, acc, g.Mm + (size_t)pos * g.T * g.K, m0, n0, wm0, wn0, lane, 0);
        }
        if (!more) break;
        acc.zero();
#pragma unroll
        for (int i = 0; i < NR; ++i) abase[i] = abase_n[i];
#pragma unroll
        for (int i = 0; i < NPB; ++i) boff[i] = boff_n[i];
        pos = pos_n; m0 = m0_n; n0 = n0_n;
        if (next_tail) in_tail = true;
        else local = nl;
    }
}

struct WinoOutArgs {
    const float* Mm;
    float* y;
    WinoGeom g;
    int K;
    int tiles_per_block;
    int do_drop;
    uint32_t drop_thresh, drop_key;
    float drop_keep;
    const pnp_step_params* sp;
    uint32_t drop_sid;
    const float* res_add;
    float* stat_ws;
    const float* stat_shift;
    const float* ep_scale;
    const float* ep_shift;
    const float* ep_res;
    int ep_cs;
    float ep_alpha;
    const float* Px;
    int tail_P, tail_F, tail_R, tail_s, tail_bn, nblk_m, nblk_n, gn;
};

template <int M, bool TS = false>
__global__ void __launch_bounds__(NT) wino_out_kernel(WinoOutArgs a) {
    constexpr int P = M + 2;
    __shared__ float red[NT * 8];
    const int K4 = a.K >> 2;
    const int kq0 = blockIdx.y * NT;
    const int K4s = (K4 - kq0) < NT ? (K4 - kq0) : NT;
    const int rpi = NT / K4s;
    const int tid = threadIdx.x;
    const int cg = tid % K4s, rsub = tid / K4s;
    const bool active = rsub < rpi;
    const int k = (kq0 + cg) * 4;
    const int t0 = blockIdx.x * a.tiles_per_block;
    int t1 = t0 + a.tiles_per_block;
    if (t1 > a.g.T) t1 = a.g.T;
    const size_t plane = (size_t)a.g.T * a.K;
    const uint32_t dkey = a.do_drop ? pnp_eff_drop_key(a.drop_key, a.sp, a.drop_sid) : 0u;
    const bool stats = a.stat_ws != nullptr;
    f32x4 s0 = {0, 0, 0, 0}, s1 = {0, 0, 0, 0};
    if (active) {
        f32x4 shift = {0, 0, 0, 0}, sc = {0, 0, 0, 0}, sh = {0, 0, 0, 0};
        if (stats && a.stat_shift) shift = ld4(a.stat_shift + k);
        if (a.ep_scale) {
            sc = ld4(a.ep_scale + k);
            sh = ld4(a.ep_shift + k);
        }
        const int cpad = (a.K - a.ep_cs) >> 1;
        for (int t = t0 + rsub; t < t1; t += rpi) {
            int n, pa, pb, ti, tj;
            tile_of(a.g, t, n, pa, pb, ti, tj);
            const float* src = a.Mm + (size_t)t * a.K + k;
            f32x4 m[P][P];
#pragma unroll
            for (int p = 0; p < P; ++p)
#pragma unroll
                for (int q = 0; q < P; ++q) m[p][q] = ld4(src + (size_t)(P * p + q) * plane);
            if constexpr (TS) {
                const int mt = t >> 7, nt = k / a.tail_bn;
                int bid;
                if (a.gn <= 0 || a.gn >= a.nblk_n) bid = mt * a.nblk_n + nt;
                else {
                    const int sc = nt / a.gn, left = a.nblk_n - sc * a.gn;
                    const int width = left < a.gn ? left : a.gn;
                    bid = sc * (a.nblk_m * a.gn) + mt * width + (nt - sc * a.gn);
                }
                const int nblk = a.nblk_m * a.nblk_n;
                int x = bid / a.tail_P, local = bid - x * a.tail_P;
                const size_t tsz = (size_t)128 * a.tail_bn;
                const size_t inner = (size_t)(t & 127) * a.tail_bn + (k - nt * a.tail_bn);
#pragma unroll
                for (int p = 0; p < P; ++p)
#pragma unroll
                    for (int q = 0; q < P; ++q) {
                        if (local >= a.tail_F) {
                            const float* px = a.Px + (size_t)(x * a.tail_R + local - a.tail_F) * (a.tail_s - 1) * tsz + inner;
                            for (int pc = 0; pc < a.tail_s - 1; ++pc) m[p][q] += ld4(px + pc * tsz);
                        }
                        local += nblk;
                        if (local >= a.tail_P) {
                            local -= a.tail_P;
                            ++x;
                        }
                    }
            }
            f32x4 o[M][M];
            if constexpr (M == 2) {
                f32x4 r[2][4];
#pragma unroll
                for (int q = 0; q < 4; ++q) {
                    r[0][q] = m[0][q] + m[1][q] + m[2][q];
                    r[1][q] = m[1][q] - m[2][q] - m[3][q];
                }
#pragma unroll
                for (int p = 0; p < 2; ++p) {
                    o[p][0] = r[p][0] + r[p][1] + r[p][2];
                    o[p][1] = r[p][1] - r[p][2] - r[p][3];
                }
            } else {
                f32x4 r[4][6];
#pragma unroll
                for (int q = 0; q < 6; ++q) {
                    f32x4 c4[4];
                    w4_at(m[0][q], m[1][q], m[2][q], m[3][q], m[4][q], m[5][q], c4);
#pragma unroll
                    for (int p = 0; p < 4; ++p) r[p][q] = c4[p];
                }
#pragma unroll
                for (int p = 0; p < 4; ++p) w4_at(r[p][0], r[p][1], r[p][2], r[p][3], r[p][4], r[p][5], o[p]);
            }
#pragma unroll
            for (int p = 0; p < M; ++p)
#pragma unroll
                for (int q = 0; q < M; ++q) {
                    const int u = M * ti + p, v = M * tj + q;
                    if (u >= a.g.Hso || v >= a.g.Wso) continue;
                    const size_t row = (size_t)(n * a.g.Ho + pa + a.g.dil * u) * a.g.Wo + pb + a.g.dil * v;
                    const size_t idx = row * a.K + k;
                    f32x4 val = o[p][q];
                    if (a.do_drop) {
#pragma unroll
                        for (int e = 0; e < 4; ++e)
                            val[e] = pnp_drop_keep((uint32_t)(idx + e), dkey, a.drop_thresh) ? val[e] / a.drop_keep : 0.f;
                    }
                    if (a.res_add) val += ld4(a.res_add + idx);
                    if (stats) {
#pragma unroll
                        for (int e = 0; e < 4; ++e) {
                            const float d = val[e] - shift[e];
                            s0[e] += d;
                            s1[e] = fmaf(d, d, s1[e]);
                        }
                    }
                    if (a.ep_scale) {
#pragma unroll
                        for (int e = 0; e < 4; ++e) val[e] = fmaf(val[e], sc[e], sh[e]);
                        if (a.ep_res) {
#pragma unroll
                            for (int e = 0; e < 4; ++e) {
                                const int cs = k + e - cpad;
                                if ((unsigned)cs < (unsigned)a.ep_cs) val[e] += a.ep_res[row * a.ep_cs + cs];
                            }
                        }
                        if (a.ep_alpha >= 0.f) {
#pragma unroll
                            for (int e = 0; e < 4; ++e) val[e] = val[e] < 0.f ? val[e] * a.ep_alpha : val[e];
                        }
                    }
                    st4(a.y + idx, val);
                }
        }
    }
    if (!stats) return;
#pragma unroll
    for (int e = 0; e < 4; ++e) {
        red[tid * 8 + e] = s0[e];
        red[tid * 8 + 4 + e] = s1[e];
    }
    __syncthreads();
    if (tid < K4s) {
        f32x4 a0 = {0, 0, 0, 0}, a1 = {0, 0, 0, 0};
        for (int j = 0; j < rpi; ++j) {
            const int tt = j * K4s + tid;
#pragma unroll
            for (int e = 0; e < 4; ++e) {
                a0[e] += red[tt * 8 + e];
                a1[e] += red[tt * 8 + 4 + e];
            }
        }
        st4(a.stat_ws + ((size_t)blockIdx.x * 2 + 0) * a.K + k, a0);
        st4(a.stat_ws + ((size_t)blockIdx.x * 2 + 1) * a.K + k, a1);
    }
}


struct WinoDyArgs {
    const float* dy;
    float* Y;
    WinoGeom g;
    int K;
};

template <int M>
__global__ void __launch_bounds__(NT) wino_dy_kernel(WinoDyArgs a) {
    const int K4 = a.K >> 2;
    const size_t nvec = (size_t)a.g.T * K4;
    const size_t plane = (size_t)a.g.T * a.K;
    const size_t gs = (size_t)gridDim.x * NT;
    for (size_t i = (size_t)blockIdx.x * NT + threadIdx.x; i < nvec; i += gs) {
        const int t = (int)(i / K4);
        const int k = (int)(i - (size_t)t * K4) * 4;
        int n, pa, pb, ti, tj;
        tile_of(a.g, t, n, pa, pb, ti, tj);
        f32x4 y[M][M];
#pragma unroll
        for (int p = 0; p < M; ++p)
#pragma unroll
            for (int q = 0; q < M; ++q) {
                const int u = M * ti + p, v = M * tj + q;
                const f32x4 zero = {0, 0, 0, 0};
                y[p][q] = (u < a.g.Hso && v < a.g.Wso) ? ld4(a.dy + ((size_t)(n * a.g.Ho + pa + a.g.dil * u) * a.g.Wo + pb + a.g.dil * v) * a.K + k) : zero;
            }
        float* out = a.Y + (size_t)t * a.K + k;
        if constexpr (M == 2) {
            f32x4 z[4][2];
#pragma unroll
            for (int q = 0; q < 2; ++q) {
                z[0][q] = y[0][q];
                z[1][q] = y[0][q] + y[1][q];
                z[2][q] = y[0][q] - y[1][q];
                z[3][q] = -y[1][q];
            }
#pragma unroll
            for (int p = 0; p < 4; ++p) {
                st4(out + (size_t)(4 * p + 0) * plane, z[p][0]);
                st4(out + (size_t)(4 * p + 1) * plane, z[p][0] + z[p][1]);
                st4(out + (size_t)(4 * p + 2) * plane, z[p][0] - z[p][1]);
// ... 385 lines not shown
}

int wgrad_split(int T, int C, int K, int npos, int* chunks_per_split) {
    const int nblk = pnp_cdiv(C, 128) * pnp_cdiv(K, 128) * npos;
    const int nchunks = pnp_cdiv(T, BK);
    static const int fixed = env_int("PNP_WINO_WGRAD_SPLIT", 0);
    int best = 1;
    double best_cost = 1e30;
    for (int ns = 1; ns <= 16; ++ns) {
        const int cps = pnp_cdiv(nchunks, ns);
        if (ns > 1 && cps < 8) break;
        if (pnp_cdiv(nchunks, cps) != ns) continue;
        const int r = pnp_cdiv((long long)nblk * ns, 256);
        const double cost = ((r / 2) * 2.0 + (r & 1) * 1.18) * (cps + 3.0) + ns * 9.4e-7 * npos * (double)C * K;
        if (cost < best_cost - 1e-9) { best_cost = cost; best = ns; }
    }
    if (fixed > 0 && pnp_cdiv(nchunks, pnp_cdiv(nchunks, fixed)) == fixed) best = fixed;
    *chunks_per_split = pnp_cdiv(nchunks, best);
    return pnp_cdiv(nchunks, *chunks_per_split);
}

struct WinoDims {
    int dtype, R, S, stride, pad_mode, dil, pad_t, pad_l, H, W, OH, OW, N, C, K;
    template <class G>
    explicit WinoDims(const G& g) : dtype(g.dtype), R(g.R), S(g.S), stride(g.stride), pad_mode(g.pad_mode), dil(g.dil), pad_t(g.pad_t), pad_l(g.pad_l), H(g.H), W(g.W), OH(g.OH), OW(g.OW), N(g.N), C(g.C), K(g.K) {}
    explicit WinoDims(const pnp_conv_geom* g) : WinoDims(*g) {}
};

WinoGeom make_wgeom(const WinoDims& d, int m) {
    WinoGeom g{};
    g.N = d.N; g.Hi = d.H; g.Wi = d.W; g.Ho = d.OH; g.Wo = d.OW; g.dil = d.dil; g.ps = d.pad_t / d.dil; g.m = m;
    g.Hsi = d.H / d.dil; g.Wsi = d.W / d.dil; g.Hso = d.OH / d.dil; g.Wso = d.OW / d.dil;
    g.th = (g.Hso + m - 1) / m; g.tw = (g.Wso + m - 1) / m;
    g.T = d.N * d.dil * d.dil * g.th * g.tw;
    return g;
}

inline size_t al256(size_t b) { return (b + 255) & ~(size_t)255; }

bool eligible_dims(const WinoDims& d, int m) {
    if (d.dtype != PNP_DTYPE_F32 || d.R != 3 || d.S != 3 || d.stride != 1 || d.pad_mode != PNP_PAD_ZERO) return false;
    if (d.dil < 1 || d.dil > 2 || d.pad_t != d.pad_l || (d.pad_t % d.dil) != 0 || d.pad_t > 2 * d.dil) return false;
    if (d.OH != d.H + 2 * d.pad_t - 2 * d.dil || d.OW != d.W + 2 * d.pad_l - 2 * d.dil) return false;
    if ((d.H % d.dil) != 0 || (d.W % d.dil) != 0 || (d.OH % d.dil) != 0 || (d.OW % d.dil) != 0) return false;
    if ((d.C % 32) != 0 || (d.K % 4) != 0 || d.K < 32) return false;
    const WinoGeom w = make_wgeom(d, m);
    const long long lim = 1ll << 29;
    return (long long)w.T * d.C < lim && (long long)w.T * d.K < lim && (long long)d.C * d.K < lim;
}

inline int gemm_bn(int K) { return K <= 64 ? 64 : 128; }

int plan_tile(const WinoDims& d, bool wgrad) {
    const int C = d.C, K = d.K;
    const int mode = wgrad ? wino_wgrad_switch.get() : wino_switch.get();
    if (mode <= 0 || wino_switch.get() <= 0) return 0;
    static const double thr2 = env_dbl("PNP_WINOGRAD_MIN", 85.0), thr2w = env_dbl("PNP_WINOGRAD_WGRAD_MIN", 120.0);
    static const double thr4 = env_dbl("PNP_WINOGRAD4_MIN", 60.0), thr4w = env_dbl("PNP_WINOGRAD4_WGRAD_MIN", 60.0);
    static const int tmin2 = env_int("PNP_WINOGRAD_TMIN", 512), tmin4 = env_int("PNP_WINOGRAD4_TMIN", 128);
    static const int wgmin = env_int("PNP_WINOGRAD_WGMIN", 256), c4max = env_int("PNP_WINOGRAD4_CMAX", 1024);
    static const double thr4lo = env_dbl("PNP_WINOGRAD4_LOW", 32.0);
    const double ck = (double)C * K / ((double)C + K);
    for (int m = wino_tile_max(); m >= 2; m -= 2) {
        if (!eligible_dims(d, m)) continue;
        const WinoGeom w = make_wgeom(d, m);
        if (m == 4 && !wgrad && C > c4max && !use_x3(w.T, C, K)) continue;
        if (mode >= 2) return m;
        if (w.T < (m == 4 ? tmin4 : tmin2)) continue;
        const long long nwg = (long long)(m + 2) * (m + 2) * pnp_cdiv(w.T, 128) * pnp_cdiv(K, gemm_bn(K));
        const double thr = m == 4 ? (wgrad ? thr4w : thr4) : (wgrad ? thr2w : thr2);
        if (ck < thr) {
            if (m != 4 || ck < thr4lo) continue;
            if (wgrad ? w.T > 32768 : nwg < 4096) continue;
        }
        if (!wgrad && nwg < (ck < 85.0 ? 2 * wgmin : wgmin)) continue;
        return m;
    }
    return 0;
}

}

namespace pnpconv {

static GemmPlan gemm_plan(int T, int C, int K, int NP, int bn, bool x3, bool xcd) {
    static const int persist = env_int("PNP_WINO_PERSIST", 1), split_on = env_int("PNP_WINO_TAILSPLIT", 0);
    GemmPlan p{};
    const long long ntiles = (long long)NP * pnp_cdiv(T, 128) * pnp_cdiv(K, bn);
    p.whole = (double)NP * T * C * 4.0 < 2147483648.0 && (double)NP * C * K * 4.0 < 2147483648.0;
    p.grid = (int)ntiles;
    p.P = (int)ntiles; p.F = (int)ntiles; p.R = 0; p.s = 1; p.px_bytes = 0;
    if (!(persist && p.whole && ntiles > 512)) return p;
    p.grid = 512;
    if (!(xcd && split_on) || x3 || (ntiles % 8) != 0) return p;
    const int P = (int)(ntiles / 8), F = (P / 64) * 64, R = P - F, ncc = C / BK;
    p.P = P; p.F = F; p.R = R;
    if (R == 0) return p;
    for (int c = 8; c >= 2; c >>= 1)
        if (c * R <= 64 && (ncc % c) == 0 && ncc / c >= 2) {
            p.s = c;
            break;
        }
    if (p.s > 1) p.px_bytes = al256((size_t)8 * R * (p.s - 1) * 128 * bn * 4);
    return p;
}

struct WinoPlan {
    int m;
    WinoGeom g;
    bool x3;
    size_t eb;
    int bn;
    bool xcd;
    GemmPlan gemm;
    int gn;
    size_t off_v, off_m, off_px, total;
    int tiles_per_block, slabs;
};
static WinoPlan plan_wino(const WinoDims& d, bool xcd) {
    static const int gn = env_int("PNP_WINO_GN", -1);
    WinoPlan p{};
    p.m = plan_tile(d, false);
    if (!p.m) return p;
    p.g = make_wgeom(d, p.m);
    const int T = p.g.T, np = (p.m + 2) * (p.m + 2);
    p.x3 = use_x3(T, d.C, d.K);
    p.eb = p.x3 ? 6 : 4;
    p.bn = gemm_bn(d.K);
    p.xcd = xcd;
    p.gemm = gemm_plan(T, d.C, d.K, np, p.bn, p.x3, xcd);
    p.gn = gn;
    p.off_v = al256((size_t)np * d.C * d.K * p.eb);
    p.off_m = p.off_v + al256((size_t)np * T * d.C * p.eb);
    p.off_px = p.off_m + al256((size_t)np * T * d.K * 4);
    p.total = p.off_px + p.gemm.px_bytes;
    const int K4 = d.K >> 2, rpi = NT / (K4 < NT ? K4 : NT);
    int iters = pnp_cdiv(T, (long long)rpi * 1024);
    if (iters < 1) iters = 1;
    p.tiles_per_block = rpi * iters;
    p.slabs = pnp_cdiv(T, p.tiles_per_block);
    return p;
}

WinoQuery wino_query(const pnp_conv_geom* g) {
    const WinoPlan p = plan_wino(WinoDims(g), true);
    return {p.m, p.total, p.slabs};
}

template <int M>
static int launch_wino_m(const ConvArgs& a, const WinoPlan& p, int kind, bool flip_transpose, void* ws, size_t ws_bytes, hipStream_t st) {
    constexpr int NP = (M + 2) * (M + 2);
    const WinoGeom& w = p.g;
    const bool x3 = p.x3, xcd = p.xcd;
    const size_t eb = p.eb;
    const GemmPlan& plan = p.gemm;
    if (!ws || ws_bytes < p.total) {
        pnp_set_error("launch_wino: workspace too small (%zu < %zu)", ws_bytes, p.total);
        return PNP_EWORKSPACE;
    }
    PNP_REQUIRE(a.y_h == nullptr && a.o_s == 0 && a.ups == 1, "launch_wino: unsupported epilogue");
    bool run_filter;
    float* U = filter_slot(a.w, flip_transpose ? 1 : 0, M, a.C, a.K, x3 ? 1 : 0, (size_t)NP * a.C * a.K * eb, (float*)ws, st, &run_filter);
    float* V = (float*)((char*)ws + p.off_v);
    float* Mm = (float*)((char*)ws + p.off_m);
    float* Px = (float*)((char*)ws + p.off_px);
    const int gn = p.gn >= 0 ? p.gn : a.gn;
    const int cls = prof_class(kind);
    if (run_filter) {
        dim3 grid((unsigned)pnp_cdiv(a.K, 32), (unsigned)pnp_cdiv(a.C, 32));
        PnpProfScope ps(cls, st, 0.0, (36.0 + eb * NP) * a.C * a.K, "wino_filter_kernel<%s, %d, %s>", flip_transpose ? "true" : "false", M, x3 ? "true" : "false");
        if (x3) {
            if (flip_transpose) hipLaunchKernelGGL((wino_filter_kernel<true, M, true>), grid, dim3(NT), 0, st, a.w, U, a.C, a.K);
            else hipLaunchKernelGGL((wino_filter_kernel<false, M, true>), grid, dim3(NT), 0, st, a.w, U, a.C, a.K);
        } else if (flip_transpose) hipLaunchKernelGGL((wino_filter_kernel<true, M, false>), grid, dim3(NT), 0, st, a.w, U, a.C, a.K);
        else hipLaunchKernelGGL((wino_filter_kernel<false, M, false>), grid, dim3(NT), 0, st, a.w, U, a.C, a.K);
        PNP_CHECK_LAUNCH("wino_filter_kernel");
    }
    {
        WinoInArgs ia{};
        ia.x = a.x; ia.V = V; ia.g = w; ia.C = a.C; ia.x_bytes = a.x_bytes; ia.xcd = a.xcd_swizzle ? env_xcd_in() : 0;
        const size_t nvec = (size_t)w.T * (a.C / 4);
        long long nb = (long long)((nvec + NT - 1) / NT);
        if (nb > 65536) nb = 65536;
        PnpProfScope ps(cls, st, 0.0, 4.0 * (double)a.N * a.H * a.W * a.C + (double)eb * NP * w.T * a.C, "wino_in_kernel<%d, %s>", M, x3 ? "true" : "false");
        if (x3) hipLaunchKernelGGL((wino_in_kernel<M, true>), dim3((unsigned)nb), dim3(NT), 0, st, ia);
        else hipLaunchKernelGGL((wino_in_kernel<M, false>), dim3((unsigned)nb), dim3(NT), 0, st, ia);
        PNP_CHECK_LAUNCH("wino_in_kernel");
    }
    if (x3) {
        const int rc = launch_wino_gemm_x3((const unsigned short*)V, (const unsigned short*)U, Mm, w.T, a.C, a.K, NP, (M == 4 ? 2 : 0) + (kind != 0), gn, xcd ? 1 : 0, 1,
                                           a.C / 32, st);
        if (rc != PNP_OK) return rc;
    } else {
        WinoGemmArgs ga{};
        ga.V = V; ga.U = U; ga.Mm = Mm; ga.T = w.T; ga.C = a.C; ga.K = a.K;
        const bool narrow = p.bn == 64;
        ga.nblk_m = pnp_cdiv(w.T, 128); ga.nblk_n = pnp_cdiv(a.K, p.bn);
        ga.gn = gn; ga.xcd_swizzle = xcd ? 2 : 0;
        ga.npos = NP;
        ga.whole = plan.whole ? 1 : 0;
        ga.tail_F = plan.F; ga.tail_R = plan.R; ga.tail_s = plan.s; ga.Px = Px;
        dim3 grid((unsigned)plan.grid);
        const double fl = 2.0 * NP * (double)w.T * a.C * a.K;
        const double by = 4.0 * NP * ((double)w.T * a.C + (double)a.C * a.K + (double)w.T * a.K);
        constexpr int KB = M == 4 ? 2 : 0;
        PnpProfScope ps(cls, st, fl, by, "wino_gemm_kernel<128, %d, 2, 2, %d>", narrow ? 64 : 128, KB + (kind != 0));
        if (narrow) {
            if (kind == 0) hipLaunchKernelGGL((wino_gemm_kernel<128, 64, 2, 2, KB>), grid, dim3(NTHREADS), 0, st, ga);
            else hipLaunchKernelGGL((wino_gemm_kernel<128, 64, 2, 2, KB + 1>), grid, dim3(NTHREADS), 0, st, ga);
        } else if (kind == 0) hipLaunchKernelGGL((wino_gemm_kernel<128, 128, 2, 2, KB>), grid, dim3(NTHREADS), 0, st, ga);
        else hipLaunchKernelGGL((wino_gemm_kernel<128, 128, 2, 2, KB + 1>), grid, dim3(NTHREADS), 0, st, ga);
        PNP_CHECK_LAUNCH("wino_gemm_kernel");
    }
    {
        WinoOutArgs oa{};
        oa.Mm = Mm; oa.y = a.y; oa.g = w; oa.K = a.K; oa.tiles_per_block = p.tiles_per_block;
        oa.do_drop = a.do_drop; oa.drop_thresh = a.drop_thresh; oa.drop_key = a.drop_key; oa.drop_keep = a.drop_keep;
        oa.sp = a.sp; oa.drop_sid = a.drop_sid;
        oa.res_add = a.res_add; oa.stat_ws = a.stat_ws; oa.stat_shift = a.stat_shift;
        oa.ep_scale = a.ep_scale; oa.ep_shift = a.ep_shift; oa.ep_res = a.ep_res; oa.ep_cs = a.ep_cs; oa.ep_alpha = a.ep_alpha;
        oa.Px = Px; oa.tail_P = plan.P; oa.tail_F = plan.F; oa.tail_R = plan.R; oa.tail_s = plan.s; oa.tail_bn = p.bn;
        oa.nblk_m = pnp_cdiv(w.T, 128); oa.nblk_n = pnp_cdiv(a.K, p.bn); oa.gn = gn;
        dim3 grid((unsigned)p.slabs, (unsigned)pnp_cdiv(a.K / 4, NT));
        PnpProfScope ps(cls, st, 0.0, 4.0 * ((double)NP * w.T * a.K + (double)a.M * a.K), "wino_out_kernel<%d>", M);
        if (oa.tail_s > 1) hipLaunchKernelGGL((wino_out_kernel<M, true>), grid, dim3(NT), 0, st, oa);
        else hipLaunchKernelGGL((wino_out_kernel<M, false>), grid, dim3(NT), 0, st, oa);
        PNP_CHECK_LAUNCH("wino_out_kernel");
    }
    return PNP_OK;
}

int launch_wino(const ConvArgs& a, int kind, bool flip_transpose, void* ws, size_t ws_bytes, hipStream_t st) {
    static const int xcd_mode = env_int("PNP_WINO_XCD", 2);
    const WinoPlan p = plan_wino(WinoDims(a), a.xcd_swizzle && xcd_mode);
    PNP_REQUIRE(p.m == 2 || p.m == 4, "launch_wino: the planner does not route this layer (policy changed between the query and the launch?)");
    return p.m == 4 ? launch_wino_m<4>(a, p, kind, flip_transpose, ws, ws_bytes, st) : launch_wino_m<2>(a, p, kind, flip_transpose, ws, ws_bytes, st);
}

inline int x3_tp(int T) { return (T + 63) & ~63; }
inline bool use_x3_wgrad(int T, int C, int K) {
    static const int on = env_int("PNP_WINOGRAD_X3_WGRAD", 1), tmin = env_int("PNP_WINOGRAD_X3_WGRAD_TMIN", 256), tmax = env_int("PNP_WINOGRAD_X3_WGRAD_TMAX", 2048);
    const int m = wino_x3_switch.get();
    if (!on || m == 0 || !wino_x3_dims_ok(C, x3_tp(T), K) || !wino_x3_dims_ok(K, x3_tp(T), C)) return false;
    return m >= 2 || (T >= tmin && T <= tmax);
}
int wgrad_split_x3(int T, int C, int K, int npos, int* sps) {
    const int nchunks = x3_tp(T) / 64;
    const long long tiles = (long long)pnp_cdiv(C, 128) * pnp_cdiv(K, gemm_bn(K)) * npos;
    int best = 1;
    double best_cost = 1e30;
    for (int ns = 1; ns <= 32 && ns <= nchunks; ++ns) {
        const int cps = pnp_cdiv(nchunks, ns);
        if (pnp_cdiv(nchunks, cps) != ns) continue;
        if (ns > 1 && cps < 2) break;
        const int rounds = pnp_cdiv(tiles * ns, 256);
        const double cost = rounds * (2.0 * cps + 3.0) + ns * 1.5e-6 * npos * (double)C * K;
        if (cost < best_cost - 1e-9) { best_cost = cost; best = ns; }
    }
    const int cps = pnp_cdiv(nchunks, best);
    *sps = 2 * cps;
    return pnp_cdiv(nchunks, cps);
}

struct WinoWgradPlan {
    int m;
    WinoGeom g;
    bool x3;
    int ns, per_split;
    int tp;
    size_t off_y, off_s, total;
    bool splitsum;
};
static WinoWgradPlan plan_wino_wgrad(const WinoDims& d) {
    WinoWgradPlan p{};
    p.m = plan_tile(d, true);
    if (!p.m) return p;
    p.g = make_wgeom(d, p.m);
    const int np = (p.m + 2) * (p.m + 2), T = p.g.T;
    p.x3 = use_x3_wgrad(T, d.C, d.K);
    p.ns = p.x3 ? wgrad_split_x3(T, d.C, d.K, np, &p.per_split) : wgrad_split(T, d.C, d.K, np, &p.per_split);
    p.tp = p.x3 ? x3_tp(T) : T;
    const size_t eb = p.x3 ? 6 : 4;
    p.off_y = al256((size_t)np * p.tp * d.C * eb);
    p.off_s = p.off_y + al256((size_t)np * p.tp * d.K * eb);
    p.total = p.off_s + al256((size_t)p.ns * np * d.C * d.K * 4);
    p.splitsum = p.ns > 2 && (size_t)d.C * (d.K / 4) < (size_t)NT * 512;
    return p;
}

WinoQuery wino_wgrad_query(const pnp_conv_geom* g) {
    const WinoWgradPlan p = plan_wino_wgrad(WinoDims(g));
    return {p.m, p.total, 0};
}

template <int M>
static int launch_wino_wgrad_m(const ConvArgs& a, const WinoWgradPlan& p, float* dw, int accumulate, void* ws, size_t ws_bytes, hipStream_t st) {
    constexpr int NP = (M + 2) * (M + 2);
    const WinoGeom& w = p.g;
    const int ns = p.ns;
    if (!ws || ws_bytes < p.total) {
        pnp_set_error("launch_wino_wgrad: workspace too small (%zu < %zu)", ws_bytes, p.total);
        return PNP_EWORKSPACE;
    }
// ... 120 lines not shown
```

### medical-cross-modality-domain-adaptation_amd/csrc/conv_x3_direct.hip

```cpp
#include "conv_x3_common.h"

using namespace pnpconv;

namespace {

constexpr int TH = 16, TW = 16, PH = TH + 2, PW = TW + 2, NPX = PH * PW;
constexpr int ROWB = 64;
constexpr int PLANE_P = NPX * ROWB;
constexpr int PATCH = 3 * PLANE_P;
constexpr int NF = 3;
constexpr int LDS_BYTES = 2 * PATCH + NF * 3 * 64 * ROWB;
constexpr int NPL = 192;
constexpr int NPI = (NPX * 8 + NPL - 1) / NPL;

__device__ __forceinline__ int swz(int row) { return (row >> 2) & 3; }

struct X3dArgs {
    const float* x;
    const unsigned short* w3;
    float* y;
    int N, H, W, C, K, OH, OW, pad_t, pad_l;
    int M;
    int do_drop;
    uint32_t drop_thresh, drop_key;
// ... 597 lines not shown
    if (ns != g->R * g->S) return false;
    p.nitems = items;
    p.taps.ngroups = p.ngroups; p.taps.R = g->R; p.taps.S = g->S;
    if (x3d_switch.get() < 2 && (items < 256 || !(g->R * g->S >= 4 * s * s || (kind == 1 && Cin <= 64)))) return false;
    if (pl) *pl = p;
    return true;
}

template <class Launch>
unsigned short* filter_image(const char* who, const char* kernel, int cls, bool flip, size_t fbytes, void* ws, size_t ws_bytes, hipStream_t st, int& rc, Launch&& launch) {
    rc = PNP_EWORKSPACE;
    if (!ws || ws_bytes < fbytes) {
        pnp_set_error("%s: workspace too small (%zu < %zu)", who, ws_bytes, fbytes);
        return nullptr;
    }
    const long long total = (long long)(fbytes / 6);
    PnpProfScope ps(cls, st, 0.0, 4.0 * total + 6.0 * total, "%s<%s>", kernel, flip ? "true" : "false");
    launch((unsigned short*)ws, dim3((unsigned)pnp_cdiv(total, 256)));
    const hipError_t e = hipGetLastError();
    if (e != hipSuccess) {
        pnp_set_error("%s: launch failed: %s", kernel, hipGetErrorString(e));
        rc = PNP_ELAUNCH;
        return nullptr;
    }
    rc = PNP_OK;
    return (unsigned short*)ws;
}

}

namespace pnpconv {

int x3d_route_mode() { return x3d_switch.get(); }

bool x3s_chosen(const pnp_conv_geom* g, int kind) { return x3s_plan(g, kind, nullptr); }

size_t x3s_filter_bytes(const pnp_conv_geom* g) { return (size_t)g->R * g->S * g->C * g->K * 6; }

int launch_x3_strided(const ConvArgs& a, const pnp_conv_geom* g, int kind, void* ws, size_t ws_bytes, hipStream_t st) {
    X3sPlan pl;
    if (!x3s_plan(g, kind, &pl)) {
        pnp_set_error("launch_x3_strided: layer not on this route");
        return PNP_EINVAL;
    }
    const size_t fbytes = x3s_filter_bytes(g);
    const int cls = prof_class(kind);
    const int Cin = kind == 0 ? g->C : g->K, Kout = kind == 0 ? g->K : g->C;
    int rc;
    unsigned short* w3 = filter_image("launch_x3_strided", "x3s_filter_kernel", cls, kind != 0, fbytes, ws, ws_bytes, st, rc, [&](unsigned short* img, dim3 blocks) {
        if (kind) hipLaunchKernelGGL((x3s_filter_kernel<true>), blocks, dim3(256), 0, st, a.w, img, Cin, Kout, pl.taps);
        else hipLaunchKernelGGL((x3s_filter_kernel<false>), blocks, dim3(256), 0, st, a.w, img, Cin, Kout, pl.taps);
    });
    if (!w3) return rc;
    X3sArgs x{};
    x.x = a.x; x.w3 = w3; x.y = a.y;
    x.N = g->N; x.C = Cin; x.K = Kout; x.NH = Cin / 32;
    if (kind == 0) { x.H = g->H; x.W = g->W; x.si = g->stride; x.OHt = g->OH; x.OWt = g->OW; x.o_s = 1; }
    else { x.H = g->OH; x.W = g->OW; x.si = 1; x.OHt = g->H; x.OWt = g->W; x.o_s = g->stride; }
    x.ngroups = pl.ngroups; x.nitems = pl.nitems;
    x.w3_bytes = (unsigned)fbytes;
    for (int i = 0; i < pl.ngroups; ++i) x.grp[i] = pl.grp[i];
    for (int i = 0; i < X3S_MAXPH; ++i) x.ph[i] = pl.ph[i];
    copy_dropout(x, a);
    x.stat_ws = kind == 0 ? a.stat_ws : nullptr; x.stat_shift = a.stat_shift;
    const dim3 grid((unsigned)(pl.nitems > 256 ? 256 : pl.nitems));
    const double fl = 6.0 * 2.0 * (double)g->N * g->OH * g->OW * g->R * g->S * g->C * g->K;
    const double by = 4.0 * ((double)g->N * x.H * x.W * Cin + (double)g->N * x.OHt * x.OWt * Kout) + 6.0 * g->R * g->S * g->C * g->K;
    PnpProfScope ps(cls, st, fl, by, "conv_x3_direct_kernel_strided<%d>", kind);
    if (kind) hipLaunchKernelGGL((conv_x3_direct_kernel_strided<1>), grid, dim3(512), 0, st, x);
    else hipLaunchKernelGGL((conv_x3_direct_kernel_strided<0>), grid, dim3(512), 0, st, x);
    PNP_CHECK_LAUNCH("conv_x3_direct_kernel_strided");
    return PNP_OK;
}

bool x3d_chosen(const pnp_conv_geom* g) {
    return x3d_switch.get() > 0 && g->dtype == PNP_DTYPE_F32 && (g->pad_mode == PNP_PAD_ZERO || (g->pad_t == 0 && g->pad_l == 0)) && dims_ok(g->R, g->S, g->stride, g->dil, g->C, g->K, g->OH, g->OW, (long long)g->N * g->OH * g->OW);
}

int x3d_stats_parts(const pnp_conv_geom* g) { return (int)(((long long)g->N * g->OH * g->OW) / 64); }

size_t x3d_filter_bytes(int C, int K) { return (size_t)9 * C * K * 6; }

int launch_x3_direct(const ConvArgs& a, int kind, bool flip_transpose, void* ws, size_t ws_bytes, hipStream_t st) {
    PNP_REQUIRE(a.ep_scale == nullptr && a.y_h == nullptr && a.o_s == 0 && a.ups == 1, "launch_x3_direct: unsupported epilogue");
    const int cls = prof_class(kind);
    const int KW = a.K == 32 ? 32 : 64;
    int rc;
    unsigned short* w3 = filter_image("launch_x3_direct", "x3d_filter_kernel", cls, flip_transpose, x3d_filter_bytes(a.C, a.K), ws, ws_bytes, st, rc, [&](unsigned short* img, dim3 blocks) {
        if (flip_transpose) hipLaunchKernelGGL((x3d_filter_kernel<true>), blocks, dim3(256), 0, st, a.w, img, a.C, a.K, KW);
        else hipLaunchKernelGGL((x3d_filter_kernel<false>), blocks, dim3(256), 0, st, a.w, img, a.C, a.K, KW);
    });
    if (!w3) return rc;
    X3dArgs x{};
    x.x = a.x; x.w3 = w3; x.y = a.y;
    x.N = a.N; x.H = a.H; x.W = a.W; x.C = a.C; x.K = a.K; x.OH = a.OH; x.OW = a.OW; x.pad_t = a.pad_t; x.pad_l = a.pad_l; x.M = a.M;
    copy_dropout(x, a);
    x.res_add = a.res_add; x.stat_ws = a.stat_ws; x.stat_shift = a.stat_shift;
    const long long nitems = (long long)a.N * (a.OH / TH) * (a.OW / TW) * (a.K / KW);
    const dim3 grid((unsigned)(nitems > 256 ? 256 : nitems));
    const double fl = 6.0 * 2.0 * (double)a.M * 9.0 * a.C * a.K;
    const double by = 4.0 * ((double)a.N * a.H * a.W * a.C + (double)a.M * a.K) + 6.0 * 9.0 * a.C * a.K;
    PnpProfScope ps(cls, st, fl, by, "conv_x3_direct_kernel<%d, %d, %d>", a.C / 32, KW, kind);
#define X3D_LAUNCH(NH_, KW_, KIND_) hipLaunchKernelGGL((conv_x3_direct_kernel<NH_, KW_, KIND_>), grid, dim3(512), 0, st, x)
    if (a.C == 32) {
        if (KW == 32) { if (kind == 0) X3D_LAUNCH(1, 32, 0); else X3D_LAUNCH(1, 32, 1); }
        else { if (kind == 0) X3D_LAUNCH(1, 64, 0); else X3D_LAUNCH(1, 64, 1); }
    } else {
        if (KW == 32) { if (kind == 0) X3D_LAUNCH(2, 32, 0); else X3D_LAUNCH(2, 32, 1); }
        else { if (kind == 0) X3D_LAUNCH(2, 64, 0); else X3D_LAUNCH(2, 64, 1); }
    }
#undef X3D_LAUNCH
    PNP_CHECK_LAUNCH("conv_x3_direct_kernel");
    return PNP_OK;
}

}

extern "C" int32_t pnp_conv2d_x3_direct(int32_t mode) { return x3d_switch.set(mode); }

extern "C" int32_t pnp_conv2d_x3_strided(int32_t mode) { return x3s_switch.set(mode); }
```

### medical-cross-modality-domain-adaptation_amd/csrc/conv_x3_narrow.hip

```cpp
#include "conv_x3_common.h"

using namespace pnpconv;

namespace {

constexpr int XC = 40, XK = 5, XR = 5;
constexpr int NCU = 256;

constexpr int F_TH = 8, F_TW = 16, F_PH = F_TH + XR - 1, F_PW = F_TW + XR - 1, F_NPX = F_PH * F_PW;
constexpr int F_PXB = 96;
constexpr int F_PLANE = F_NPX * F_PXB;
constexpr int F_TAIL = 64;
constexpr int F_PATCH = 3 * F_PLANE + F_TAIL;
constexpr int F_ROWV = F_TW * XK;
constexpr int F_RED = 4 * F_TH * F_ROWV * 4;
constexpr int F_LDS = F_PATCH + F_RED;
constexpr int F_NSLAB = 8;
constexpr size_t F_IMG = (size_t)F_NSLAB * XR * 3 * 64 * 16;

constexpr int D_T = 16, D_P = D_T + XR - 1, D_NPX = D_P * D_P;
constexpr int D_PLANE = D_NPX * 16;
constexpr int D_PATCH = 3 * D_PLANE;
constexpr int D_NSLAB = 7;
constexpr int D_FSP = XC * 64;
// ... 216 lines not shown
                    for (int rr = 0; rr < 4; ++rr) {
                        bf16x8 xf[3];
#pragma unroll
                        for (int p = 0; p < 3; ++p)
                            xf[p] = *reinterpret_cast<const bf16x8*>(patch + p * D_PLANE + ((4 * wave + rr) * D_P + p16) * 16 + toff[j]);
#pragma unroll
                        for (int blk = 0; blk < 3; ++blk)
#pragma unroll
                            for (int trm = 0; trm < (kX3nAblate == 1 ? 0 : 6); ++trm)
                                acc[rr][blk] = __builtin_amdgcn_mfma_f32_16x16x32_bf16(wf[blk][kTermW[trm]], xf[kTermX[trm]], acc[rr][blk], 0, 0, 0);
                    }
                }
#pragma unroll
                for (int rr = 0; rr < 4; ++rr) {
                    const int oh = oh0 + 4 * wave + rr, ow = ow0 + p16;
#pragma unroll
                    for (int blk = 0; blk < 3; ++blk) {
                        const int ch = 16 * blk + 4 * g;
                        if (oh < a.OH && ow < a.OW && ch < XC) {
                            const size_t off = (((size_t)n * a.OH + oh) * a.OW + ow) * XC + ch;
                            f32x4 v = acc[rr][blk];
                            if (a.res_add) v += *reinterpret_cast<const f32x4*>(a.res_add + off);
                            *reinterpret_cast<f32x4*>(a.y + off) = v;
                        }
                    }
                }
            }
            __syncthreads();
        }
    }
}

template <bool FLIP>
__global__ void __launch_bounds__(256) x3n_filter_kernel(const float* __restrict__ w, unsigned short* __restrict__ w3) {
    const int i = blockIdx.x * 256 + threadIdx.x;
    float v = 0.f;
    size_t base, pstride;
    if (!FLIP) {
        if (i >= F_NSLAB * XR * 64 * 8) return;
        const int e = i & 7, lane = (i >> 3) & 63, sr = i >> 9;
        const int r = sr % XR, slab = sr / XR;
        const int row = lane & 15, q = 32 * slab + 8 * (lane >> 4) + e;
        const int s = q / 48, ch = q - s * 48;
        if (row < XK && s < XR && ch < XC) v = w[((size_t)(r * XR + s) * XC + ch) * XK + row];
        base = ((size_t)((slab * XR + r) * 3) * 64 + lane) * 8 + e;
        pstride = 64 * 8;
    } else {
        if (i >= D_NSLAB * XC * 32) return;
        const int kk = i & 31, row = (i >> 5) % XC, j = (i >> 5) / XC;
        const int tp = 4 * j + (kk >> 3), e = kk & 7;
        if (tp < XR * XR && e < XK) v = w[((size_t)(XR * XR - 1 - tp) * XC + row) * XK + e];
        base = ((size_t)(j * 3) * XC + row) * 32 + kk;
        pstride = (size_t)XC * 32;
    }
    split3_write(w3 + base, pstride, v);
}

ModeSwitch x3n_switch{"PNP_X3_NARROW", 1, 2, false};

constexpr bool kShips[2] = {true, true};

long long x3n_items(const pnp_conv_geom* g, int kind) {
    return kind == 0 ? (long long)g->N * (g->OH / F_TH) * (g->OW / F_TW) : (long long)g->N * pnp_cdiv(g->H, D_T) * pnp_cdiv(g->W, D_T);
}

}

namespace pnpconv {

bool x3n_chosen(const pnp_conv_geom* g, int kind) {
    const int mode = x3n_switch.get();
    if (x3d_route_mode() <= 0 || mode <= 0) return false;
    if (g->dtype != PNP_DTYPE_F32 || g->pad_mode != PNP_PAD_ZERO || g->R != XR || g->S != XR || g->stride != 1 || g->dil != 1 || g->C != XC || g->K != XK)
        return false;
    if (g->pad_t < 0 || g->pad_l < 0 || g->pad_t > XR - 1 || g->pad_l > XR - 1 || g->OH <= 0 || g->OW <= 0) return false;
    if ((long long)g->N * g->H * g->W * XC >= (1ll << 30) || (long long)g->N * g->OH * g->OW * XK >= (1ll << 30)) return false;
    if (kind == 0 && ((g->OH % F_TH) != 0 || (g->OW % F_TW) != 0)) return false;
    return mode >= 2 || (kShips[kind != 0] && x3n_items(g, kind) >= 256);
}

size_t x3n_filter_bytes(int kind) { return kind == 0 ? F_IMG : (size_t)D_FILT; }

int launch_x3_narrow(const ConvArgs& a, int kind, void* ws, size_t ws_bytes, hipStream_t st) {
    PNP_REQUIRE(a.ep_scale == nullptr && a.y_h == nullptr && a.o_s == 0 && a.ups == 1 && a.stat_ws == nullptr, "launch_x3_narrow: unsupported epilogue");
    PNP_REQUIRE(a.R == XR && a.S == XR && a.C == (kind ? XK : XC) && a.K == (kind ? XC : XK) && (kind || ((a.OH % F_TH) == 0 && (a.OW % F_TW) == 0)),
                "launch_x3_narrow: layer not on this route");
    const size_t fbytes = x3n_filter_bytes(kind);
    if (!ws || ws_bytes < fbytes) {
        pnp_set_error("launch_x3_narrow: workspace too small (%zu < %zu)", ws_bytes, fbytes);
        return PNP_EWORKSPACE;
    }
    unsigned short* w3 = (unsigned short*)ws;
    const int cls = prof_class(kind);
    const int total = XR * XR * XC * XK;
    {
        PnpProfScope ps(cls, st, 0.0, 4.0 * total + (double)fbytes, "x3n_filter_kernel<%s>", kind ? "true" : "false");
        if (kind) hipLaunchKernelGGL((x3n_filter_kernel<true>), dim3((unsigned)pnp_cdiv(D_NSLAB * XC * 32, 256)), dim3(256), 0, st, a.w, w3);
        else hipLaunchKernelGGL((x3n_filter_kernel<false>), dim3((unsigned)pnp_cdiv(F_NSLAB * XR * 64 * 8, 256)), dim3(256), 0, st, a.w, w3);
        PNP_CHECK_LAUNCH("x3n_filter_kernel");
    }
    X3nArgs x{};
    x.x = a.x; x.w3 = w3; x.y = a.y; x.res_add = kind ? a.res_add : nullptr;
    x.N = a.N; x.H = a.H; x.W = a.W; x.OH = a.OH; x.OW = a.OW; x.pad_t = a.pad_t; x.pad_l = a.pad_l;
    x.tiles_x = kind ? pnp_cdiv(a.OW, D_T) : a.OW / F_TW;
    x.tiles_y = kind ? pnp_cdiv(a.OH, D_T) : a.OH / F_TH;
    const long long nitems = (long long)a.N * x.tiles_x * x.tiles_y;
    x.nitems = (int)nitems;
    copy_dropout(x, a);
    const dim3 grid((unsigned)(nitems > 2 * NCU ? 2 * NCU : nitems));
    const double fl = 6.0 * 2.0 * (double)a.M * XR * XR * XC * XK;
    const double by = 4.0 * ((double)a.N * a.H * a.W * a.C + (double)a.M * a.K) + (double)fbytes;
    PnpProfScope ps(cls, st, fl, by, "conv_x3_direct_kernel_narrow<%d>", kind);
    if (kind) hipLaunchKernelGGL((conv_x3_direct_kernel_narrow<1>), grid, dim3(256), 0, st, x);
    else hipLaunchKernelGGL((conv_x3_direct_kernel_narrow<0>), grid, dim3(256), 0, st, x);
    PNP_CHECK_LAUNCH("conv_x3_direct_kernel_narrow");
    return PNP_OK;
}

}

extern "C" int32_t pnp_conv2d_x3_narrow(int32_t mode) { return x3n_switch.set(mode); }
```

### medical-cross-modality-domain-adaptation_amd/csrc/pnp_common.h

```cpp
#pragma once
#include <hip/hip_runtime.h>
#include <stdint.h>
#include <stdio.h>
#include <stdlib.h>
#include "pnp_hip.h"

typedef float f32x16 __attribute__((ext_vector_type(16)));
typedef float f32x4 __attribute__((ext_vector_type(4)));

constexpr int MAXC = 8;

void pnp_set_error(const char* fmt, ...);

#define PNP_CHECK_LAUNCH(name)                                                   \
    do {                                                                         \
        hipError_t e__ = hipGetLastError();                                      \
        if (e__ != hipSuccess) {                                                 \
            pnp_set_error("%s: launch failed: %s", name, hipGetErrorString(e__)); \
            return PNP_ELAUNCH;                                                  \
        }                                                                        \
    } while (0)

#define PNP_REQUIRE(cond, ...)            \
    do {                                  \
        if (!(cond)) {                    \
            pnp_set_error(__VA_ARGS__);   \
            return PNP_EINVAL;            \
        }                                 \
    } while (0)

__host__ __device__ __forceinline__ uint32_t pnp_fmix32(uint32_t h) {
    h ^= h >> 16;
    h *= 0x85EBCA6Bu;
    h ^= h >> 13;
    h *= 0xC2B2AE35u;
    h ^= h >> 16;
    return h;
}
__host__ __device__ __forceinline__ uint32_t pnp_drop_key(uint64_t seed, uint32_t stream_id) {
    uint32_t lo = (uint32_t)seed, hi = (uint32_t)(seed >> 32);
    uint32_t k = pnp_fmix32(hi + 0x9E3779B9u * (stream_id + 1u));
    return pnp_fmix32(lo ^ k);
}
__host__ __device__ __forceinline__ uint32_t pnp_drop_thresh(float keep) {
    double t = (1.0 - (double)keep) * 16777216.0 + 0.5;
    if (t < 0) t = 0;
    if (t > 16777216.0) t = 16777216.0;
    return (uint32_t)t;
}
__host__ __device__ __forceinline__ bool pnp_drop_keep(uint32_t idx, uint32_t key, uint32_t thresh) {
    uint32_t h = pnp_fmix32((idx * 0xCC9E2D51u) ^ key);
    return (h >> 8) >= thresh;
}

struct pnp_step_params {
    unsigned long long drop_seed;
    float adam_lr_t;
    float reserved;
};
const pnp_step_params* pnp_step_params_ptr();
__device__ __forceinline__ uint32_t pnp_eff_drop_key(uint32_t key, const pnp_step_params* sp, uint32_t stream_id) {
    return sp ? pnp_drop_key(sp->drop_seed, stream_id) : key;
}

struct PnpProfScope {
    PnpProfScope(int cls, hipStream_t st, double flops, double bytes, const char* fmt, ...) __attribute__((format(printf, 6, 7)));
    ~PnpProfScope();
    PnpProfScope(const PnpProfScope&) = delete;
    bool on_;
    hipStream_t st_;
    hipEvent_t e0_, e1_;
    double flops_, bytes_;
    char name_[128];
};

static inline int pnp_cdiv(long long a, long long b) { return (int)((a + b - 1) / b); }
```

### medical-cross-modality-domain-adaptation_amd/functional.py

```python
import os

import torch
from torch.autograd import Function

from . import _lib
from . import gradsink
from . import kernels as K
from . import parallel as par

BN_EPS = 1e-3
BN_DECAY = 0.90
LEAK = 0.2
FUSE_BN_INFER = os.environ.get("PNP_FUSE_BN_INFER", "1") != "0"
FUSE_BN_STATS = os.environ.get("PNP_FUSE_BN_STATS", "1") != "0"
BN_RECOMPUTE_SIGN = os.environ.get("PNP_BN_RECOMPUTE_SIGN", "1") != "0"
PS_FUSE = os.environ.get("PNP_PS_FUSE", "1") != "0"


def sync_now():
    return par.sync_world() > 1 and torch.is_grad_enabled()


_STAT_VERSION = {}

# ... 137 lines not shown
    if ctx.is_train and ctx.P_norm != xc.numel() // xc.shape[-1]:
        sums = K.bn_bwd_reduce(dout, out, xc, mean, var, BN_EPS, ctx.alpha, gamma, beta)
        gsums = par.all_sum_(sums.clone())
        dxc, dsc = K.bn_bwd_apply(dout, out, xc, mean, var, gamma, gsums, ctx.P_norm, need_sc, BN_EPS, ctx.alpha, True, keep, seed, sid,
                                  beta=beta, want_h=want_h, only_h=only_h)
        dgamma, dbeta = sums[0], sums[1]
        if slots is not None:
            K.axpby(dgamma, slots[0], 1.0, 1.0)
            K.axpby(dbeta, slots[1], 1.0, 1.0)
    else:
        dxc, dgamma, dbeta, dsc = K.bn_bwd(dout, out, xc, mean, var, gamma, need_sc, BN_EPS, ctx.alpha, ctx.is_train, keep, seed, sid,
                                           into=slots, beta=beta, want_h=want_h, only_h=only_h)
    if slots is not None:
        gradsink.done(sinks[0])
        gradsink.done(sinks[1])
        return dxc, None, None, dsc
    return dxc, dgamma, dbeta, dsc


def _bn_sinks(ctx, gamma, beta, ig, ib, taped=True):
    ctx.bn_sinks = None
    if taped and ctx.needs_input_grad[ig] and ctx.needs_input_grad[ib]:
        sg, sb = gradsink.lookup(gamma), gradsink.lookup(beta)
        if sg is not None and sb is not None:
            sg.pending += 1
            sb.pending += 1
            ctx.bn_sinks = (sg, sb)


class Conv2dDropFn(Function):
    @staticmethod
    def forward(ctx, x, w, geom, keep_prob, seed, stream_id, taped=True):
        x = _contig(x)
        w_ = _contig(w)
        ctx.xh = None
        if K.bf16r(geom, 0):
            xh = K.bf16_of(x)
            y = K.conv2d_fwd_bf16r(xh, K.filter_shadows(w_)[1], geom, keep_prob, seed, stream_id)[0]
            if taped and ctx.needs_input_grad[1] and K.bf16r(geom, 2):
                ctx.xh = xh
        else:
            y = K.conv2d_fwd(x, w_, geom, keep_prob, seed, stream_id)
        ctx.save_for_backward(x, w_)
        ctx.geom, ctx.keep, ctx.seed, ctx.sid = geom, keep_prob, seed, stream_id
        ctx.w_sink = gradsink.use(w_, taped) if ctx.needs_input_grad[1] else None
        return y

    @staticmethod
    def backward(ctx, dy):
        x, w = ctx.saved_tensors
        dy = _contig(dy)
        if ctx.keep < 1.0:
            dy = K.dropout(dy, ctx.keep, ctx.seed, ctx.sid, want_h=_bwd_wants_h(ctx))
        dx = _dgrad(ctx, dy, w) if ctx.needs_input_grad[0] else None
        dw = _wgrad(ctx, x, dy, ctx.w_sink) if ctx.needs_input_grad[1] else None
        return dx, dw, None, None, None, None, None


class ConvBNActFn(Function):

    @staticmethod
    def forward(ctx, x, w, gamma, beta, moving_mean, moving_var, shortcut, geom, keep_prob, seed, stream_id, is_train, alpha, sync=False,
                link=None, taped=True):
        x = _contig(x)
        w_ = _contig(w)
        sc = _contig(shortcut) if shortcut is not None else None
        ctx.geom, ctx.keep, ctx.seed, ctx.sid = geom, keep_prob, seed, stream_id
        ctx.is_train, ctx.alpha = is_train, alpha
        ctx.sc_channels = sc.shape[-1] if sc is not None else 0
        ctx.link = link if RES_LINK else None
        ctx.w_sink = gradsink.use(w_, taped) if ctx.needs_input_grad[1] else None
        _bn_sinks(ctx, gamma, beta, 2, 3, taped)
        ctx.fused = (not is_train) and FUSE_BN_INFER and (not taped or not (ctx.needs_input_grad[2] or ctx.needs_input_grad[3]))
        res = K.bf16r(geom, 0)
        ctx.xh = None
        h_mode = geom.dtype == _lib.DTYPE_BF16
        if res:
            xh = K.bf16_of(x)
            w_oi = K.filter_shadows(w_)[1]
            if taped and ctx.needs_input_grad[1] and K.bf16r(geom, 2):
                ctx.xh = xh
        if ctx.fused:
            mean, var = _frozen_stats(ctx, moving_mean, moving_var)
            ss = K.bn_fold(gamma, beta, mean, var, BN_EPS)
            if res:
                out, outh, _ = K.conv2d_fwd_bf16r(xh, w_oi, geom, keep_prob, seed, stream_id, want_h=True, bn=(ss, sc, alpha))
                K.set_bf16(out, outh)
            else:
                out = K.conv2d_fwd_bn(x, w_, geom, ss, sc, alpha, keep_prob, seed, stream_id)
            ctx.P_norm = out.numel() // out.shape[-1]
            ctx.save_for_backward(x, w_, out, out, mean, var, gamma)
            return out
        P = geom.N * geom.OH * geom.OW
        ctx.P_norm = P
        parts = None
        if res:
            xc, _, parts = K.conv2d_fwd_bf16r(xh, w_oi, geom, keep_prob, seed, stream_id, stat_shift=moving_mean,
                                              want_stats=is_train and FUSE_BN_STATS)
        elif is_train and FUSE_BN_STATS and K.conv_stats_parts(geom) > 0:
            xc, parts = K.conv2d_fwd_stats(x, w_, geom, moving_mean, keep_prob, seed, stream_id)
        else:
            xc = K.conv2d_fwd(x, w_, geom, keep_prob, seed, stream_id)
        if is_train:
            if sync:
                local = K.bn_stats_finish(parts, moving_mean, P) if parts is not None else K.bn_stats(xc)
                mean, var = par.sync_bn_stats(*local)
                ctx.P_norm = P * par.sync_world()
                K.bn_update_moving(moving_mean, moving_var, mean, var, ctx.P_norm, BN_DECAY)
            elif parts is not None:
                mean, var = K.bn_stats_finish(parts, moving_mean, P, moving_mean, moving_var, BN_DECAY)
            else:
                mean, var = K.bn_stats_update(xc, moving_mean, moving_var, BN_DECAY)
            _bump_stat_version(moving_mean, moving_var)
        else:
            mean, var = _frozen_stats(ctx, moving_mean, moving_var)
        out = K.bn_apply(xc, mean, var, gamma, beta, sc, BN_EPS, alpha, want_h=h_mode)
        ctx.resign = BN_RECOMPUTE_SIGN and sc is None and alpha >= 0.0
        ctx.wepoch = K._WEIGHT_EPOCH[0]
        ctx.save_for_backward(x, w_, xc, beta if ctx.resign else out, mean, var, gamma)
        return out

    @staticmethod
    def backward(ctx, dout):
        x, w, xc, out, mean, var, gamma = ctx.saved_tensors
        beta = None
        if getattr(ctx, "resign", False):
            if ctx.wepoch != K._WEIGHT_EPOCH[0]:
                raise RuntimeError("parameters were updated (optimiser / clip / load) between a forward pass and its backward pass: the "
                                   "BN backward recomputes the activation's sign from gamma / beta and would use the NEW values "
                                   "(set PNP_BN_RECOMPUTE_SIGN=0 for flows that step between forward and backward)")
            out, beta = None, out
        _check_frozen_stats(ctx, mean, var)
        dout = _contig(dout)
        need_sc = ctx.sc_channels if ctx.needs_input_grad[6] else 0
        want_h = _bwd_wants_h(ctx)
        only_h = _bwd_only_h(ctx)
        if ctx.fused:
            dxc, dsc = K.bn_bwd_apply(dout, out, out, mean, var, gamma, None, ctx.P_norm, need_sc, BN_EPS, ctx.alpha, False, ctx.keep,
                                      ctx.seed, ctx.sid, want_h=want_h, only_h=only_h)
            dgamma = dbeta = None
        else:
            dxc, dgamma, dbeta, dsc = _bn_bwd(ctx, dout, out, xc, mean, var, gamma, need_sc, ctx.keep, ctx.seed, ctx.sid, beta, want_h, only_h)
        res = None
        if ctx.link is not None:
            if ctx.sc_channels:
                ctx.link.dsc, dsc = dsc, None
            else:
                res = ctx.link.take()
        if ctx.needs_input_grad[0]:
            dx = _dgrad(ctx, dxc, w, residual=res)
        else:
            dx = None
        dw = _wgrad(ctx, x, dxc, ctx.w_sink) if ctx.needs_input_grad[1] else None
        return (dx, dw, dgamma if ctx.needs_input_grad[2] else None, dbeta if ctx.needs_input_grad[3] else None, None, None,
                dsc, None, None, None, None, None, None, None, None, None)


class BNActFn(Function):

    @staticmethod
    def forward(ctx, xc, gamma, beta, moving_mean, moving_var, is_train, alpha, sync=False, taped=True):
        xc = _contig(xc)
        P = xc.numel() // xc.shape[-1]
        ctx.P_norm = P
        _bn_sinks(ctx, gamma, beta, 1, 2, taped)
        if is_train:
            if sync:
                mean, var = par.sync_bn_stats(*K.bn_stats(xc))
                ctx.P_norm = P * par.sync_world()
                K.bn_update_moving(moving_mean, moving_var, mean, var, ctx.P_norm, BN_DECAY)
            else:
# ... 217 lines not shown
```

### medical-cross-modality-domain-adaptation_amd/kernels.py

```python
import ctypes
import os
import weakref

import torch

from . import _lib
from ._lib import ConvGeom, PAD_SYMMETRIC, PAD_ZERO, check

_ws_cache = {}


_raw_stream = getattr(torch._C, "_cuda_getCurrentRawStream", None)
_raw_device = getattr(torch._C, "_cuda_getDevice", None)


def _stream_ptr():
    if _raw_stream is not None and _raw_device is not None:
        return _raw_stream(_raw_device())
    return torch.cuda.current_stream().cuda_stream


def _stream():
    return ctypes.c_void_p(_stream_ptr())

# ... 64 lines not shown
        g.OH = (H - ((R - 1) * dil + 1)) // stride + 1
        g.OW = (W - ((S - 1) * dil + 1)) // stride + 1
        g.pad_mode = PAD_ZERO
    else:
        raise ValueError("unknown padding %r" % (padding,))
    return g


def conv2d_fwd(x, w, g, keep_prob=1.0, seed=0, stream_id=0, out=None, naive=False):
    lib = _lib.load()
    y = out if out is not None else torch.empty((g.N, g.OH, g.OW, g.K), dtype=torch.float32, device=x.device)
    if naive:
        check(lib.pnp_conv2d_fwd_naive(_p(x), _p(w), _p(y), ctypes.byref(g), _stream()), "pnp_conv2d_fwd_naive")
    else:
        nbytes = lib.pnp_conv2d_fwd_workspace_bytes(ctypes.byref(g))
        ws = workspace(nbytes, x.device) if nbytes else None
        _wino_u(w, g, 0)
        check(lib.pnp_conv2d_fwd_ws(_p(x), _p(w), _p(y), ctypes.byref(g), float(keep_prob), int(seed), int(stream_id),
                                    ctypes.c_void_p(ws.data_ptr()) if ws is not None else None, ws.numel() if ws is not None else 0,
                                    _stream()), "pnp_conv2d_fwd")
    return y


def conv_stats_parts(g):
    return int(_lib.load().pnp_conv2d_fwd_stats_ws_parts(ctypes.byref(g)))


def wino_mode(mode=-1):
    return int(_lib.load().pnp_conv2d_wino_mode(int(mode)))


def wino_wgrad_mode(mode=-1):
    return int(_lib.load().pnp_conv2d_wino_wgrad_mode(int(mode)))


def wino_tile(tile=-1):
    return int(_lib.load().pnp_conv2d_wino_tile(int(tile)))


def wino_x3(mode=-1):
    return int(_lib.load().pnp_conv2d_wino_x3(int(mode)))


def x3_direct(mode=-1):
    return int(_lib.load().pnp_conv2d_x3_direct(int(mode)))


def x3_strided(mode=-1):
    return int(_lib.load().pnp_conv2d_x3_strided(int(mode)))


def x3_wgrad(mode=-1):
    return int(_lib.load().pnp_conv2d_x3_wgrad(int(mode)))


def x3_narrow(mode=-1):
    return int(_lib.load().pnp_conv2d_x3_narrow(int(mode)))


def wino_chosen(g, kind=0):
    return int(_lib.load().pnp_conv2d_wino_chosen(ctypes.byref(g), int(kind)))


def conv_route(g, kind=0):
    return int(_lib.load().pnp_conv2d_route(ctypes.byref(g), int(kind)))


U_CACHE = os.environ.get("PNP_WINOGRAD_UCACHE", "1") != "0"
_u_cache = {}


def _u_drop(key, ref=None):
    ent = _u_cache.get(key)
    if ent is None or (ref is not None and ent[0] is not ref):
        return
    del _u_cache[key]
    if ent[1] is not None:
        try:
            _lib.load().pnp_conv2d_wino_filter_bind(ctypes.c_void_p(key[0]), int(key[1]), None, 0)
        except Exception:
            pass


def _wino_u(w, g, kind):
    if not U_CACHE:
        return
    key = (w.data_ptr(), kind)
    ent = _u_cache.get(key)
    if not getattr(w, "_pnp_var", False):
        if ent is not None:
            _u_drop(key)
        return
    if ent is not None and ent[0]() is w:
        if ent[2] != w._version:
            if ent[1] is not None:
                _lib.load().pnp_weights_changed(ctypes.c_void_p(w.data_ptr()), ctypes.c_void_p(w.data_ptr() + 4 * w.numel()))
            ent[2] = w._version
        if ent[1] is not None or not (g.R == 3 and g.S == 3 and wino_chosen(g, kind)):
            return
    lib = _lib.load()
    if ent is not None and not (ent[0]() is w and ent[1] is None):
        _u_drop(key)
    U = None
    if g.R == 3 and g.S == 3 and wino_chosen(g, kind):
        nbytes = int(lib.pnp_conv2d_wino_filter_bytes(int(w.shape[2]), int(w.shape[3])))
        if nbytes:
            U = torch.empty(nbytes // 4, dtype=torch.float32, device=w.device)
            check(lib.pnp_conv2d_wino_filter_bind(ctypes.c_void_p(w.data_ptr()), int(kind), ctypes.c_void_p(U.data_ptr()), nbytes),
                  "pnp_conv2d_wino_filter_bind")
    _u_cache[key] = [weakref.ref(w, lambda r, k=key: _u_drop(k, r)), U, w._version]


def wino_u_cache_clear():
    if _u_cache:
        _lib.load().pnp_conv2d_wino_filter_bind(None, 0, None, 0)
        _u_cache.clear()


def memory_report():
    nb = lambda t: 0 if t is None else int(t.numel()) * int(t.element_size())
    rep = {"workspaces": sum(nb(b) for b in _ws_cache.values()), "workspace_buffers": len(_ws_cache),
           "workspaces_retired": sum(nb(b) for b in _ws_retired), "recorded_steps_alive": int(PINNED[0]),
           "winograd_filters": sum(nb(e[1]) for e in _u_cache.values()), "winograd_filter_entries": len(_u_cache),
           "bf16_filter_shadows": sum(nb(e[1]) + nb(e[2]) for e in _filter_cache.values()), "bf16_filter_entries": len(_filter_cache)}
    rep["total"] = rep["workspaces"] + rep["workspaces_retired"] + rep["winograd_filters"] + rep["bf16_filter_shadows"]
    return rep


def wino_u_cache_stats(reset=False):
    h, f = ctypes.c_int64(0), ctypes.c_int64(0)
    _lib.load().pnp_conv2d_wino_filter_stats(ctypes.byref(h), ctypes.byref(f), 1 if reset else 0)
    return int(h.value), int(f.value)


def _fwd_ws(g, device):
    nbytes = _lib.load().pnp_conv2d_fwd_workspace_bytes(ctypes.byref(g))
    if not nbytes:
        return None, 0
    ws = workspace(nbytes, device)
    return ctypes.c_void_p(ws.data_ptr()), ws.numel()


def conv2d_fwd_stats(x, w, g, shift, keep_prob=1.0, seed=0, stream_id=0):
    lib = _lib.load()
    nparts = conv_stats_parts(g)
    y = torch.empty((g.N, g.OH, g.OW, g.K), dtype=torch.float32, device=x.device)
    parts = workspace(nparts * 2 * g.K * 4, x.device, slot="stats")
    wsp, wsn = _fwd_ws(g, x.device)
    _wino_u(w, g, 0)
    check(lib.pnp_conv2d_fwd_stats_ws(_p(x), _p(w), _p(y), ctypes.byref(g), float(keep_prob), int(seed), int(stream_id), _p(shift),
                                      ctypes.c_void_p(parts.data_ptr()), parts.numel(), wsp, wsn, _stream()), "pnp_conv2d_fwd_stats_ws")
    return y, (parts, nparts)


def bn_stats_finish(parts_n, shift, P, mm=None, mv=None, decay=0.9):
    parts, nparts = parts_n
    C = shift.numel()
    mean = torch.empty(C, dtype=torch.float32, device=shift.device)
    var = torch.empty(C, dtype=torch.float32, device=shift.device)
    check(_lib.load().pnp_bn_stats_finish(ctypes.c_void_p(parts.data_ptr()), int(nparts), _p(shift), _p(mean), _p(var), _p(mm), _p(mv), int(P), C,
                                          float(decay), _stream()), "pnp_bn_stats_finish")
    return mean, var


def bn_fold(gamma, beta, mean, var, eps=1e-3):
    lib = _lib.load()
    C = gamma.numel()
    ss = torch.empty((2, C), dtype=torch.float32, device=gamma.device)
    check(lib.pnp_bn_fold(_p(gamma), _p(beta), _p(mean), _p(var), _p(ss[0]), _p(ss[1]), C, float(eps), _stream()), "pnp_bn_fold")
    return ss


def conv2d_fwd_bn(x, w, g, scale_shift, shortcut=None, alpha=0.2, keep_prob=1.0, seed=0, stream_id=0):
    lib = _lib.load()
    y = torch.empty((g.N, g.OH, g.OW, g.K), dtype=torch.float32, device=x.device)
    cs = shortcut.shape[-1] if shortcut is not None else 0
    wsp, wsn = _fwd_ws(g, x.device)
    _wino_u(w, g, 0)
    check(lib.pnp_conv2d_fwd_bn_ws(_p(x), _p(w), _p(y), ctypes.byref(g), float(keep_prob), int(seed), int(stream_id), _p(scale_shift[0]),
                                   _p(scale_shift[1]), _p(shortcut), cs, float(alpha), wsp, wsn, _stream()), "pnp_conv2d_fwd_bn_ws")
    return y


def cast_bf16(x):
    y = torch.empty(x.shape, dtype=torch.bfloat16, device=x.device)
    check(_lib.load().pnp_cast_bf16(_p(x), _ph(y), x.numel(), _stream()), "pnp_cast_bf16")
    return y


def filter_bf16(w, want_io=True, want_oi=True):
    R, S, C, Kc = w.shape
    w_io = torch.empty((R * S, C, Kc), dtype=torch.bfloat16, device=w.device) if want_io else None
    w_oi = torch.empty((R * S, Kc, C), dtype=torch.bfloat16, device=w.device) if want_oi else None
    check(_lib.load().pnp_filter_bf16(_p(w), _ph(w_io), _ph(w_oi), R, S, C, Kc, _stream()), "pnp_filter_bf16")
    return w_io, w_oi


_WEIGHT_EPOCH = [0]
_CHANGES = []
_CHANGE_FLOOR = [0]
_filter_cache = {}
CAST_COUNT = [0]


RECORDING = [None]
PINNED = [0]


def weights_changed(ranges=None):
    _WEIGHT_EPOCH[0] += 1
    if ranges is None or len(_CHANGES) >= 64:
        _CHANGES.clear()
        _CHANGE_FLOOR[0] = _WEIGHT_EPOCH[0]
    else:
        _CHANGES.append((_WEIGHT_EPOCH[0], tuple((int(lo), int(hi)) for lo, hi in ranges)))
    if len(_filter_cache) > 1024 and not PINNED[0]:
        _filter_cache.clear()
    if _u_cache:
        lib = _lib.load()
        if ranges is None and len(_u_cache) > 4096 and not PINNED[0]:
            wino_u_cache_clear()
        elif ranges is None:
            lib.pnp_weights_changed(None, None)
        else:
            for lo, hi in ranges:
                lib.pnp_weights_changed(ctypes.c_void_p(lo), ctypes.c_void_p(hi))


class HalfOnly(object):
    __slots__ = ("h",)

    def __init__(self, h):
        self.h = h

    @property
    def shape(self):
        return self.h.shape


def bf16_of(t):
    if isinstance(t, HalfOnly):
        return t.h
    h = getattr(t, "_pnp_h", None)
    if h is not None and h[1] == t._version and h[0].shape == t.shape and not torch.cuda.is_current_stream_capturing():
        return h[0]
    CAST_COUNT[0] += 1
    hh = cast_bf16(t)
    set_bf16(t, hh)
    return hh


def set_bf16(t, h):
    if h is not None:
        t._pnp_h = (h, t._version)
    return t


def _changed_since(epoch, lo, hi):
    if epoch < _CHANGE_FLOOR[0]:
        return True
    for ep, rs in reversed(_CHANGES):
        if ep <= epoch:
            break
# ... 985 lines not shown
```

Before: 295.2 slices/s.

## Fold BN params into conv epilogue and cache dgrad flipped filter images

Adds a conv forward path that takes raw BN gamma/beta/mean/var and computes the scale and shift inside the kernel epilogue. On routes that support it (Winograd, N16), this removes the separate bn_fold launch. It also extends the per-weight filter-image cache so that dgrad's flip/transpose images are built once per weight version rather than on every call. In exchange there is extra cache memory, a per-thread rsqrt in the epilogue, and more Python-side route queries per layer call.

```diff
diff --git a/include/pnp_hip.h b/include/pnp_hip.h
--- a/include/pnp_hip.h
+++ b/include/pnp_hip.h
@@ -88,6 +88,7 @@
 size_t pnp_conv2d_wino_filter_bytes(int32_t C, int32_t K);
 int pnp_conv2d_wino_filter_bind(const float* w, int32_t kind, float* U, size_t bytes);
 void pnp_weights_changed(const void* lo, const void* hi);
+size_t pnp_conv2d_filter_image_bytes(const pnp_conv_geom* g, int32_t kind);
 void pnp_conv2d_wino_filter_stats(int64_t* hits, int64_t* fills, int32_t reset);
 int32_t pnp_conv2d_wino_wgrad_mode(int32_t mode);
 
@@ -101,6 +102,16 @@
                          float keep_prob, uint64_t seed, uint32_t stream_id,
                          const float* scale, const float* shift, const float* shortcut , int32_t Cs, float alpha,
                          void* workspace, size_t workspace_bytes, void* stream);
+int32_t pnp_conv2d_fwd_bn_params_served(const pnp_conv_geom* g, size_t workspace_bytes);
+int pnp_conv2d_fwd_bn_params(const float* x, const float* w, float* y, const pnp_conv_geom* g,
+                             float keep_prob, uint64_t seed, uint32_t stream_id,
+                             const float* gamma, const float* beta, const float* mean, const float* var, float eps,
+                             const float* shortcut , int32_t Cs, float alpha, void* stream);
+int pnp_conv2d_fwd_bn_params_ws(const float* x, const float* w, float* y, const pnp_conv_geom* g,
+                                float keep_prob, uint64_t seed, uint32_t stream_id,
+                                const float* gamma, const float* beta, const float* mean, const float* var, float eps,
+                                const float* shortcut , int32_t Cs, float alpha,
+                                void* workspace, size_t workspace_bytes, void* stream);
 
 size_t pnp_conv2d_dgrad_workspace_bytes(const pnp_conv_geom* g);
 int pnp_conv2d_dgrad(const float* dy, const float* w, float* dx, const pnp_conv_geom* g,
diff --git a/medical-cross-modality-domain-adaptation_amd/_lib.py b/medical-cross-modality-domain-adaptation_amd/_lib.py
--- a/medical-cross-modality-domain-adaptation_amd/_lib.py
+++ b/medical-cross-modality-domain-adaptation_amd/_lib.py
@@ -79,6 +79,10 @@
     "pnp_bn_fold": (c_int, [_F, _F, _F, _F, _F, _F, c_int32, c_float, c_void_p]),
     "pnp_conv2d_fwd_bn": (c_int, [_F, _F, _F, _G, c_float, c_uint64, c_uint32, _F, _F, _F, c_int32, c_float, c_void_p]),
     "pnp_conv2d_fwd_bn_ws": (c_int, [_F, _F, _F, _G, c_float, c_uint64, c_uint32, _F, _F, _F, c_int32, c_float, c_void_p, c_size_t, c_void_p]),
+    "pnp_conv2d_fwd_bn_params_served": (c_int32, [_G, c_size_t]),
+    "pnp_conv2d_fwd_bn_params": (c_int, [_F, _F, _F, _G, c_float, c_uint64, c_uint32, _F, _F, _F, _F, c_float, _F, c_int32, c_float, c_void_p]),
+    "pnp_conv2d_fwd_bn_params_ws": (c_int, [_F, _F, _F, _G, c_float, c_uint64, c_uint32, _F, _F, _F, _F, c_float, _F, c_int32, c_float, c_void_p,
+                                            c_size_t, c_void_p]),
     "pnp_conv2d_fwd_stats_ws_parts": (c_int32, [_G]),
     "pnp_conv2d_fwd_stats_ws": (c_int, [_F, _F, _F, _G, c_float, c_uint64, c_uint32, _F, _F, c_size_t, c_void_p, c_size_t, c_void_p]),
     "pnp_conv2d_wino_chosen": (c_int32, [_G, c_int32]),
@@ -95,6 +99,7 @@
     "pnp_conv2d_wino_filter_bind": (c_int, [c_void_p, c_int32, c_void_p, c_size_t]),
     "pnp_weights_changed": (None, [c_void_p, c_void_p]),
     "pnp_conv2d_wino_filter_stats": (None, [POINTER(c_int64), POINTER(c_int64), c_int32]),
+    "pnp_conv2d_filter_image_bytes": (c_size_t, [_G, c_int32]),
     "pnp_conv2d_fwd_naive": (c_int, [_F, _F, _F, _G, c_void_p]),
     "pnp_dropout": (c_int, [_F, _F, c_size_t, c_float, c_uint64, c_uint32, c_void_p]),
     "pnp_bn_workspace_bytes": (c_size_t, [c_int64, c_int32]),
diff --git a/medical-cross-modality-domain-adaptation_amd/csrc/conv_common.h b/medical-cross-modality-domain-adaptation_amd/csrc/conv_common.h
--- a/medical-cross-modality-domain-adaptation_amd/csrc/conv_common.h
+++ b/medical-cross-modality-domain-adaptation_amd/csrc/conv_common.h
@@ -33,6 +33,11 @@
     const float* ep_res;
     int ep_cs;
     float ep_alpha;
+    const float* bn_gamma;
+    const float* bn_beta;
+    const float* bn_mean;
+    const float* bn_var;
+    float bn_eps;
     int dtype;
     float* stat_ws;
     const float* stat_shift;
@@ -57,8 +62,17 @@
     }
 }
 
-__device__ __forceinline__ float bn_epilogue(const ConvArgs& a, float v, int m, int n) {
-    v = fmaf(v, a.ep_scale[n], a.ep_shift[n]);
+__device__ __forceinline__ bool ep_bn_on(const ConvArgs& a) { return a.ep_scale != nullptr || a.bn_gamma != nullptr; }
+__device__ __forceinline__ void ep_coeffs(const ConvArgs& a, int n, float& sc, float& sh) {
+    if (a.bn_gamma) pnp_bn_coeffs(a.bn_gamma[n], a.bn_beta[n], a.bn_mean[n], a.bn_var[n], a.bn_eps, sc, sh);
+    else {
+        sc = a.ep_scale[n];
+        sh = a.ep_shift[n];
+    }
+}
+
+__device__ __forceinline__ float bn_epilogue(const ConvArgs& a, float v, int m, int n, float sc, float sh) {
+    v = fmaf(v, sc, sh);
     if (a.ep_res) {
         const int cs = n - ((a.K - a.ep_cs) >> 1);
         if ((unsigned)cs < (unsigned)a.ep_cs) v += a.ep_res[(size_t)m * a.ep_cs + cs];
@@ -342,6 +356,9 @@
     int stats_parts;
 };
 WinoQuery wino_query(const pnp_conv_geom* g);
+enum FilterImageFmt { FI_U = 0, FI_U3 = 1, FI_FLIP = 2, FI_PHASES = 3 };
+inline int filter_shape_code(int R, int S, int stride) { return (R << 16) | (S << 8) | stride; }
+float* filter_image_slot(const float* w, int kind, int fmt, int shape, int C, int K, size_t need, float* ws_img, hipStream_t st, bool* run);
 int launch_wino(const ConvArgs& a, int kind, bool flip_transpose, void* ws, size_t ws_bytes, hipStream_t st);
 WinoQuery wino_wgrad_query(const pnp_conv_geom* g);
 int launch_wino_wgrad(const ConvArgs& a, float* dw, int accumulate, void* ws, size_t ws_bytes, hipStream_t st);
diff --git a/medical-cross-modality-domain-adaptation_amd/csrc/conv_igemm.hip b/medical-cross-modality-domain-adaptation_amd/csrc/conv_igemm.hip
--- a/medical-cross-modality-domain-adaptation_amd/csrc/conv_igemm.hip
+++ b/medical-cross-modality-domain-adaptation_amd/csrc/conv_igemm.hip
@@ -872,9 +872,10 @@
                                const float* __restrict__ var, float* __restrict__ scale, float* __restrict__ shift, int C, float eps) {
     const int c = blockIdx.x * blockDim.x + threadIdx.x;
     if (c >= C) return;
-    const float sc = gamma[c] * (1.0f / sqrtf(var[c] + eps));
+    float sc, sh;
+    pnp_bn_coeffs(gamma[c], beta[c], mean[c], var[c], eps, sc, sh);
     scale[c] = sc;
-    shift[c] = beta[c] - mean[c] * sc;
+    shift[c] = sh;
 }
 
 __global__ void flip_transpose_phase_kernel(const float* __restrict__ w, float* __restrict__ wt, int R, int S, int C, int K, int st) {
@@ -1563,6 +1564,15 @@
 size_t pnp_conv2d_dgrad_workspace_bytes(const pnp_conv_geom* g) { return g ? plan_dgrad(g).ws_bytes : 0; }
 size_t pnp_conv2d_wgrad_workspace_bytes(const pnp_conv_geom* g) { return g ? plan_wgrad(g).ws_bytes : 0; }
 
+size_t pnp_conv2d_filter_image_bytes(const pnp_conv_geom* g, int32_t kind) {
+    if (!g || (kind != 0 && kind != 1) || check_geom(g, "pnp_conv2d_filter_image_bytes") != PNP_OK) return 0;
+    const int route = plan_of(g, kind).cand[0].route;
+    if (route == PNP_ROUTE_WINO) return pnp_conv2d_wino_filter_bytes(g->C, g->K);
+    if (kind == 1 && (route == PNP_ROUTE_PHASES || route == PNP_ROUTE_IGEMM || route == PNP_ROUTE_N16 || route == PNP_ROUTE_NARROW))
+        return (size_t)g->R * g->S * g->C * g->K * sizeof(float);
+    return 0;
+}
+
 int pnp_conv2d_fwd(const float* x, const float* w, float* y, const pnp_conv_geom* g, float keep_prob, uint64_t seed,
                    uint32_t stream_id, void* stream) {
     return pnp_conv2d_fwd_ws(x, w, y, g, keep_prob, seed, stream_id, nullptr, 0, stream);
@@ -1633,17 +1643,54 @@
     return pnp_conv2d_fwd_bn_ws(x, w, y, g, keep_prob, seed, stream_id, scale, shift, shortcut, Cs, alpha, nullptr, 0, stream);
 }
 
-int pnp_conv2d_fwd_bn_ws(const float* x, const float* w, float* y, const pnp_conv_geom* g, float keep_prob, uint64_t seed,
-                         uint32_t stream_id, const float* scale, const float* shift, const float* shortcut, int32_t Cs, float alpha,
-                         void* workspace, size_t workspace_bytes, void* stream) {
+static bool bn_params_route(int route) { return route == PNP_ROUTE_WINO || route == PNP_ROUTE_N16; }
+
+int32_t pnp_conv2d_fwd_bn_params_served(const pnp_conv_geom* g, size_t workspace_bytes) {
+    if (!g || check_geom(g, "pnp_conv2d_fwd_bn_params_served") != PNP_OK) return 0;
+    const void* have = workspace_bytes ? (const void*)g : nullptr;
+    return bn_params_route(plan_fwd(g, EP_WS | EP_BN).pick(have, workspace_bytes).route) ? 1 : 0;
+}
+
+static int fwd_bn_impl(const float* x, const float* w, float* y, const pnp_conv_geom* g, float keep_prob, uint64_t seed, uint32_t stream_id,
+                       const ConvArgs& bn, const float* shortcut, int32_t Cs, float alpha, void* workspace, size_t workspace_bytes, void* stream) {
     if (int e = check_geom(g, "pnp_conv2d_fwd_bn")) return e;
-    PNP_REQUIRE(x && w && y && scale && shift, "pnp_conv2d_fwd_bn: null pointer");
+    PNP_REQUIRE(x && w && y, "pnp_conv2d_fwd_bn: null pointer");
     PNP_REQUIRE(keep_prob > 0.f, "pnp_conv2d_fwd_bn: keep_prob must be > 0");
     if (shortcut) PNP_REQUIRE(Cs > 0 && Cs <= g->K && ((g->K - Cs) % 2) == 0, "pnp_conv2d_fwd_bn: bad shortcut channels");
     ConvArgs a = make_args(x, w, y, g);
     set_dropout(a, keep_prob, seed, stream_id);
-    a.ep_scale = scale; a.ep_shift = shift; a.ep_res = shortcut; a.ep_cs = shortcut ? Cs : g->K; a.ep_alpha = alpha;
-    return launch_fwd_cand(plan_fwd(g, EP_WS | EP_BN).pick(workspace, workspace_bytes), a, g, workspace, workspace_bytes, (hipStream_t)stream);
+    a.ep_scale = bn.ep_scale; a.ep_shift = bn.ep_shift;
+    a.bn_gamma = bn.bn_gamma; a.bn_beta = bn.bn_beta; a.bn_mean = bn.bn_mean; a.bn_var = bn.bn_var; a.bn_eps = bn.bn_eps;
+    a.ep_res = shortcut; a.ep_cs = shortcut ? Cs : g->K; a.ep_alpha = alpha;
+    const ConvPlan p = plan_fwd(g, EP_WS | EP_BN);
+    const ConvPlan::Cand& c = p.pick(workspace, workspace_bytes);
+    PNP_REQUIRE(!bn.bn_gamma || bn_params_route(c.route),
+                "pnp_conv2d_fwd_bn_params: this layer's kernel takes folded coefficients (pnp_conv2d_fwd_bn_params_served == 0): pnp_bn_fold + pnp_conv2d_fwd_bn");
+    return launch_fwd_cand(c, a, g, workspace, workspace_bytes, (hipStream_t)stream);
+}
+
+int pnp_conv2d_fwd_bn_ws(const float* x, const float* w, float* y, const pnp_conv_geom* g, float keep_prob, uint64_t seed,
+                         uint32_t stream_id, const float* scale, const float* shift, const float* shortcut, int32_t Cs, float alpha,
+                         void* workspace, size_t workspace_bytes, void* stream) {
+    PNP_REQUIRE(scale && shift, "pnp_conv2d_fwd_bn: null pointer");
+    ConvArgs bn{};
+    bn.ep_scale = scale; bn.ep_shift = shift;
+    return fwd_bn_impl(x, w, y, g, keep_prob, seed, stream_id, bn, shortcut, Cs, alpha, workspace, workspace_bytes, stream);
+}
+
+int pnp_conv2d_fwd_bn_params(const float* x, const float* w, float* y, const pnp_conv_geom* g, float keep_prob, uint64_t seed,
+                             uint32_t stream_id, const float* gamma, const float* beta, const float* mean, const float* var, float eps,
+                             const float* shortcut, int32_t Cs, float alpha, void* stream) {
+    return pnp_conv2d_fwd_bn_params_ws(x, w, y, g, keep_prob, seed, stream_id, gamma, beta, mean, var, eps, shortcut, Cs, alpha, nullptr, 0, stream);
+}
+
+int pnp_conv2d_fwd_bn_params_ws(const float* x, const float* w, float* y, const pnp_conv_geom* g, float keep_prob, uint64_t seed,
+                                uint32_t stream_id, const float* gamma, const float* beta, const float* mean, const float* var, float eps,
+                                const float* shortcut, int32_t Cs, float alpha, void* workspace, size_t workspace_bytes, void* stream) {
+    PNP_REQUIRE(gamma && beta && mean && var, "pnp_conv2d_fwd_bn_params: null pointer");
+    ConvArgs bn{};
+    bn.bn_gamma = gamma; bn.bn_beta = beta; bn.bn_mean = mean; bn.bn_var = var; bn.bn_eps = eps;
+    return fwd_bn_impl(x, w, y, g, keep_prob, seed, stream_id, bn, shortcut, Cs, alpha, workspace, workspace_bytes, stream);
 }
 
 int pnp_conv2d_fwd_naive(const float* x, const float* w, float* y, const pnp_conv_geom* g, void* stream) {
@@ -1680,7 +1727,10 @@
                                        : launch_x3_direct(a, 1, true, workspace, workspace_bytes, st);
     }
     const DgradWs& dws = p.dws;
-    float* wt = (float*)workspace;
+    const size_t img_bytes = (size_t)g->R * g->S * g->C * g->K * sizeof(float);
+    bool build = true;
+    float* wt = filter_image_slot(w, 1, route == PNP_ROUTE_PHASES ? FI_PHASES : FI_FLIP, filter_shape_code(g->R, g->S, g->stride), g->C, g->K,
+                                  img_bytes, (float*)workspace, st, &build);
     float* out = sym ? (float*)((char*)workspace + dws.filt) : dx;
     float* parts = (float*)((char*)workspace + dws.filt + dws.padded);
     auto split_ws = [&](int ns) { return ns > 1 ? parts : nullptr; };
@@ -1688,8 +1738,10 @@
     if (route == PNP_ROUTE_PHASES) {
         DgradPhase ph[16];
         const int nph = plan_phases(g, ph);
-        hipLaunchKernelGGL(flip_transpose_phase_kernel, tg, dim3(256), 0, st, w, wt, g->R, g->S, g->C, g->K, g->stride);
-        PNP_CHECK_LAUNCH("flip_transpose_phase_kernel");
+        if (build) {
+            hipLaunchKernelGGL(flip_transpose_phase_kernel, tg, dim3(256), 0, st, w, wt, g->R, g->S, g->C, g->K, g->stride);
+            PNP_CHECK_LAUNCH("flip_transpose_phase_kernel");
+        }
         if (phases_in_one_launch(g, ph, nph)) {
             if (int e = launch_phase_group(dy, wt, out, g, ph, nph, d.OH, d.OW, st)) return e;
         } else {
@@ -1703,8 +1755,10 @@
             }
         }
     } else {
-        hipLaunchKernelGGL(flip_transpose_kernel, tg, dim3(256), 0, st, w, wt, g->R, g->S, g->C, g->K);
-        PNP_CHECK_LAUNCH("flip_transpose_kernel");
+        if (build) {
+            hipLaunchKernelGGL(flip_transpose_kernel, tg, dim3(256), 0, st, w, wt, g->R, g->S, g->C, g->K);
+            PNP_CHECK_LAUNCH("flip_transpose_kernel");
+        }
         PNP_REQUIRE(d.pad_t >= 0 && d.pad_l >= 0, "pnp_conv2d_dgrad: forward padding exceeds the filter extent");
         ConvArgs a = make_args(dy, wt, out, &d);
         a.ups = g->stride;
diff --git a/medical-cross-modality-domain-adaptation_amd/csrc/conv_small.hip b/medical-cross-modality-domain-adaptation_amd/csrc/conv_small.hip
--- a/medical-cross-modality-domain-adaptation_amd/csrc/conv_small.hip
+++ b/medical-cross-modality-domain-adaptation_amd/csrc/conv_small.hip
@@ -31,6 +31,9 @@
     const int p = lane & 15, g = lane >> 4;
     const int n = blockIdx.z, oh0 = blockIdx.y * TH;
     const __amdgpu_buffer_rsrc_t rx = make_rsrc(a.x, a.x_bytes);
+    const bool ep_bn = ep_bn_on(a);
+    float ep_sc = 0.f, ep_sh = 0.f;
+    if (ep_bn) ep_coeffs(a, p, ep_sc, ep_sh);
 
     float wreg[9][NH][4];
 #pragma unroll
@@ -78,7 +81,7 @@
                 float v = acc[q][i];
                 if (a.do_drop) v = pnp_drop_keep((uint32_t)oidx[q][i], pnp_eff_drop_key(a.drop_key, a.sp, a.drop_sid), a.drop_thresh) ? v / a.drop_keep : 0.f;
                 if (a.res_add) v += a.res_add[oidx[q][i]];
-                if (a.ep_scale) v = bn_epilogue(a, v, m, p);
+                if (ep_bn) v = bn_epilogue(a, v, m, p, ep_sc, ep_sh);
                 ov[q][i] = v;
             }
         }
@@ -179,6 +182,9 @@
     const int p = lane & 15, g = lane >> 4;
     const int n = blockIdx.z, oh0 = blockIdx.y * TH;
     const __amdgpu_buffer_rsrc_t rx = make_rsrc(a.x, a.x_bytes);
+    const bool ep_bn = ep_bn_on(a);
+    float ep_sc = 0.f, ep_sh = 0.f;
+    if (ep_bn) ep_coeffs(a, p, ep_sc, ep_sh);
     float wreg[7];
     int aoff[7];
 #pragma unroll
@@ -213,7 +219,7 @@
                 float v = acc[i];
                 if (a.do_drop) v = pnp_drop_keep((uint32_t)oidx[i], pnp_eff_drop_key(a.drop_key, a.sp, a.drop_sid), a.drop_thresh) ? v / a.drop_keep : 0.f;
                 if (a.res_add) v += a.res_add[oidx[i]];
-                if (a.ep_scale) v = bn_epilogue(a, v, m, p);
+                if (ep_bn) v = bn_epilogue(a, v, m, p, ep_sc, ep_sh);
                 ov[i] = v;
             }
 #pragma unroll
diff --git a/medical-cross-modality-domain-adaptation_amd/csrc/conv_wino.hip b/medical-cross-modality-domain-adaptation_amd/csrc/conv_wino.hip
--- a/medical-cross-modality-domain-adaptation_amd/csrc/conv_wino.hip
+++ b/medical-cross-modality-domain-adaptation_amd/csrc/conv_wino.hip
@@ -412,6 +412,11 @@
     const float* ep_res;
     int ep_cs;
     float ep_alpha;
+    const float* bn_gamma;
+    const float* bn_beta;
+    const float* bn_mean;
+    const float* bn_var;
+    float bn_eps;
     const float* Px;
     int tail_P, tail_F, tail_R, tail_s, tail_bn, nblk_m, nblk_n, gn;
 };
@@ -438,7 +443,17 @@
     if (active) {
         f32x4 shift = {0, 0, 0, 0}, sc = {0, 0, 0, 0}, sh = {0, 0, 0, 0};
         if (stats && a.stat_shift) shift = ld4(a.stat_shift + k);
-        if (a.ep_scale) {
+        const bool ep_bn = a.ep_scale != nullptr || a.bn_gamma != nullptr;
+        if (a.bn_gamma) {
+            const f32x4 ga = ld4(a.bn_gamma + k), be = ld4(a.bn_beta + k), mu = ld4(a.bn_mean + k), va = ld4(a.bn_var + k);
+#pragma unroll
+            for (int e = 0; e < 4; ++e) {
+                float s, t;
+                pnp_bn_coeffs(ga[e], be[e], mu[e], va[e], a.bn_eps, s, t);
+                sc[e] = s;
+                sh[e] = t;
+            }
+        } else if (a.ep_scale) {
             sc = ld4(a.ep_scale + k);
             sh = ld4(a.ep_shift + k);
         }
@@ -528,7 +543,7 @@
                             s1[e] = fmaf(d, d, s1[e]);
                         }
                     }
-                    if (a.ep_scale) {
+                    if (ep_bn) {
 #pragma unroll
                         for (int e = 0; e < 4; ++e) val[e] = fmaf(val[e], sc[e], sh[e]);
                         if (a.ep_res) {
@@ -1080,6 +1095,10 @@
 }
 
 namespace pnpconv {
+
+float* filter_image_slot(const float* w, int kind, int fmt, int shape, int C, int K, size_t need, float* ws_img, hipStream_t st, bool* run) {
+    return filter_slot(w, kind, shape, C, K, fmt, need, ws_img, st, run);
+}
 
 static GemmPlan gemm_plan(int T, int C, int K, int NP, int bn, bool x3, bool xcd) {
     static const int persist = env_int("PNP_WINO_PERSIST", 1), split_on = env_int("PNP_WINO_TAILSPLIT", 0);
@@ -1217,6 +1236,7 @@
         oa.sp = a.sp; oa.drop_sid = a.drop_sid;
         oa.res_add = a.res_add; oa.stat_ws = a.stat_ws; oa.stat_shift = a.stat_shift;
         oa.ep_scale = a.ep_scale; oa.ep_shift = a.ep_shift; oa.ep_res = a.ep_res; oa.ep_cs = a.ep_cs; oa.ep_alpha = a.ep_alpha;
+        oa.bn_gamma = a.bn_gamma; oa.bn_beta = a.bn_beta; oa.bn_mean = a.bn_mean; oa.bn_var = a.bn_var; oa.bn_eps = a.bn_eps;
         oa.Px = Px; oa.tail_P = plan.P; oa.tail_F = plan.F; oa.tail_R = plan.R; oa.tail_s = plan.s; oa.tail_bn = p.bn;
         oa.nblk_m = pnp_cdiv(w.T, 128); oa.nblk_n = pnp_cdiv(a.K, p.bn); oa.gn = gn;
         dim3 grid((unsigned)p.slabs, (unsigned)pnp_cdiv(a.K / 4, NT));
diff --git a/medical-cross-modality-domain-adaptation_amd/csrc/conv_x3_direct.hip b/medical-cross-modality-domain-adaptation_amd/csrc/conv_x3_direct.hip
--- a/medical-cross-modality-domain-adaptation_amd/csrc/conv_x3_direct.hip
+++ b/medical-cross-modality-domain-adaptation_amd/csrc/conv_x3_direct.hip
@@ -703,7 +703,7 @@
 size_t x3d_filter_bytes(int C, int K) { return (size_t)9 * C * K * 6; }
 
 int launch_x3_direct(const ConvArgs& a, int kind, bool flip_transpose, void* ws, size_t ws_bytes, hipStream_t st) {
-    PNP_REQUIRE(a.ep_scale == nullptr && a.y_h == nullptr && a.o_s == 0 && a.ups == 1, "launch_x3_direct: unsupported epilogue");
+    PNP_REQUIRE(a.ep_scale == nullptr && a.bn_gamma == nullptr && a.y_h == nullptr && a.o_s == 0 && a.ups == 1, "launch_x3_direct: unsupported epilogue");
     const int cls = prof_class(kind);
     const int KW = a.K == 32 ? 32 : 64;
     int rc;
diff --git a/medical-cross-modality-domain-adaptation_amd/csrc/conv_x3_narrow.hip b/medical-cross-modality-domain-adaptation_amd/csrc/conv_x3_narrow.hip
--- a/medical-cross-modality-domain-adaptation_amd/csrc/conv_x3_narrow.hip
+++ b/medical-cross-modality-domain-adaptation_amd/csrc/conv_x3_narrow.hip
@@ -322,7 +322,7 @@
 size_t x3n_filter_bytes(int kind) { return kind == 0 ? F_IMG : (size_t)D_FILT; }
 
 int launch_x3_narrow(const ConvArgs& a, int kind, void* ws, size_t ws_bytes, hipStream_t st) {
-    PNP_REQUIRE(a.ep_scale == nullptr && a.y_h == nullptr && a.o_s == 0 && a.ups == 1 && a.stat_ws == nullptr, "launch_x3_narrow: unsupported epilogue");
+    PNP_REQUIRE(a.ep_scale == nullptr && a.bn_gamma == nullptr && a.y_h == nullptr && a.o_s == 0 && a.ups == 1 && a.stat_ws == nullptr, "launch_x3_narrow: unsupported epilogue");
     PNP_REQUIRE(a.R == XR && a.S == XR && a.C == (kind ? XK : XC) && a.K == (kind ? XC : XK) && (kind || ((a.OH % F_TH) == 0 && (a.OW % F_TW) == 0)),
                 "launch_x3_narrow: layer not on this route");
     const size_t fbytes = x3n_filter_bytes(kind);
diff --git a/medical-cross-modality-domain-adaptation_amd/csrc/pnp_common.h b/medical-cross-modality-domain-adaptation_amd/csrc/pnp_common.h
--- a/medical-cross-modality-domain-adaptation_amd/csrc/pnp_common.h
+++ b/medical-cross-modality-domain-adaptation_amd/csrc/pnp_common.h
@@ -63,6 +63,11 @@
     return sp ? pnp_drop_key(sp->drop_seed, stream_id) : key;
 }
 
+__device__ __forceinline__ void pnp_bn_coeffs(float gamma, float beta, float mean, float var, float eps, float& scale, float& shift) {
+    scale = gamma * (1.0f / sqrtf(var + eps));
+    shift = fmaf(-mean, scale, beta);
+}
+
 struct PnpProfScope {
     PnpProfScope(int cls, hipStream_t st, double flops, double bytes, const char* fmt, ...) __attribute__((format(printf, 6, 7)));
     ~PnpProfScope();
diff --git a/medical-cross-modality-domain-adaptation_amd/functional.py b/medical-cross-modality-domain-adaptation_amd/functional.py
--- a/medical-cross-modality-domain-adaptation_amd/functional.py
+++ b/medical-cross-modality-domain-adaptation_amd/functional.py
@@ -243,11 +243,14 @@
                 ctx.xh = xh
         if ctx.fused:
             mean, var = _frozen_stats(ctx, moving_mean, moving_var)
-            ss = K.bn_fold(gamma, beta, mean, var, BN_EPS)
-            if res:
+            if not res and K.fwd_bn_params_served(geom):
+                out = K.conv2d_fwd_bn_params(x, w_, geom, gamma, beta, mean, var, BN_EPS, sc, alpha, keep_prob, seed, stream_id)
+            elif res:
+                ss = K.bn_fold(gamma, beta, mean, var, BN_EPS)
                 out, outh, _ = K.conv2d_fwd_bf16r(xh, w_oi, geom, keep_prob, seed, stream_id, want_h=True, bn=(ss, sc, alpha))
                 K.set_bf16(out, outh)
             else:
+                ss = K.bn_fold(gamma, beta, mean, var, BN_EPS)
                 out = K.conv2d_fwd_bn(x, w_, geom, ss, sc, alpha, keep_prob, seed, stream_id)
             ctx.P_norm = out.numel() // out.shape[-1]
             ctx.save_for_backward(x, w_, out, out, mean, var, gamma)
diff --git a/medical-cross-modality-domain-adaptation_amd/kernels.py b/medical-cross-modality-domain-adaptation_amd/kernels.py
--- a/medical-cross-modality-domain-adaptation_amd/kernels.py
+++ b/medical-cross-modality-domain-adaptation_amd/kernels.py
@@ -170,6 +170,10 @@
             pass
 
 
+def _dgrad_image_bytes(g, kind):
+    return int(_lib.load().pnp_conv2d_filter_image_bytes(ctypes.byref(g), int(kind))) if kind == 1 else 0
+
+
 def _wino_u(w, g, kind):
     if not U_CACHE:
         return
@@ -184,7 +188,7 @@
             if ent[1] is not None:
                 _lib.load().pnp_weights_changed(ctypes.c_void_p(w.data_ptr()), ctypes.c_void_p(w.data_ptr() + 4 * w.numel()))
             ent[2] = w._version
-        if ent[1] is not None or not (g.R == 3 and g.S == 3 and wino_chosen(g, kind)):
+        if ent[1] is not None or not ((g.R == 3 and g.S == 3 and wino_chosen(g, kind)) or _dgrad_image_bytes(g, kind)):
             return
     lib = _lib.load()
     if ent is not None and not (ent[0]() is w and ent[1] is None):
@@ -192,10 +196,12 @@
     U = None
     if g.R == 3 and g.S == 3 and wino_chosen(g, kind):
         nbytes = int(lib.pnp_conv2d_wino_filter_bytes(int(w.shape[2]), int(w.shape[3])))
-        if nbytes:
-            U = torch.empty(nbytes // 4, dtype=torch.float32, device=w.device)
-            check(lib.pnp_conv2d_wino_filter_bind(ctypes.c_void_p(w.data_ptr()), int(kind), ctypes.c_void_p(U.data_ptr()), nbytes),
-                  "pnp_conv2d_wino_filter_bind")
+    else:
+        nbytes = _dgrad_image_bytes(g, kind)
+    if nbytes:
+        U = torch.empty(nbytes // 4, dtype=torch.float32, device=w.device)
+        check(lib.pnp_conv2d_wino_filter_bind(ctypes.c_void_p(w.data_ptr()), int(kind), ctypes.c_void_p(U.data_ptr()), nbytes),
+              "pnp_conv2d_wino_filter_bind")
     _u_cache[key] = [weakref.ref(w, lambda r, k=key: _u_drop(k, r)), U, w._version]
 
 
@@ -267,6 +273,23 @@
     _wino_u(w, g, 0)
     check(lib.pnp_conv2d_fwd_bn_ws(_p(x), _p(w), _p(y), ctypes.byref(g), float(keep_prob), int(seed), int(stream_id), _p(scale_shift[0]),
                                    _p(scale_shift[1]), _p(shortcut), cs, float(alpha), wsp, wsn, _stream()), "pnp_conv2d_fwd_bn_ws")
+    return y
+
+
+def fwd_bn_params_served(g):
+    lib = _lib.load()
+    return bool(lib.pnp_conv2d_fwd_bn_params_served(ctypes.byref(g), lib.pnp_conv2d_fwd_workspace_bytes(ctypes.byref(g))))
+
+
+def conv2d_fwd_bn_params(x, w, g, gamma, beta, mean, var, eps=1e-3, shortcut=None, alpha=0.2, keep_prob=1.0, seed=0, stream_id=0):
+    lib = _lib.load()
+    y = torch.empty((g.N, g.OH, g.OW, g.K), dtype=torch.float32, device=x.device)
+    cs = shortcut.shape[-1] if shortcut is not None else 0
+    wsp, wsn = _fwd_ws(g, x.device)
+    _wino_u(w, g, 0)
+    check(lib.pnp_conv2d_fwd_bn_params_ws(_p(x), _p(w), _p(y), ctypes.byref(g), float(keep_prob), int(seed), int(stream_id), _p(gamma), _p(beta),
+                                          _p(mean), _p(var), float(eps), _p(shortcut), cs, float(alpha), wsp, wsn, _stream()),
+          "pnp_conv2d_fwd_bn_params_ws")
     return y
 
 
```

Result: no change. 296.2 slices/s, median of 6 (+0.3%).
